# kaistmm/Audio-Mamba-AuM

Hardware: AMD Instinct MI355X
Metric: clips/sec/node AuM-Base 128x1024 fwd+bwd (higher is better)
Workload: dtype bf16; 1 GPU; AuM-Base (d_model=768, 24 Fo-Bi blocks, d_state=16, 92.1M params) 128-mel x 1024-frame clips, L=513 tokens, fwd+bwd+Adam, bf16 autocast / fp32 master weights, input = 160000-sample waveforms through the one-launch HIP frontend (log-mel + 16x16 patch embedding + position rows); per_gpu_batch=64, global_batch=64, parallelism=dp1

## Files before the change

audio-mamba-aum_amd/aum_hip/__init__.py:

```python
import ctypes as C
import math
import os

import torch

_HERE = os.path.dirname(os.path.abspath(__file__))
_SO = os.path.join(_HERE, "libaum_hip.so")

AUM_F32, AUM_BF16, AUM_F16 = 0, 1, 2
SCAN_SOFTPLUS, SCAN_REVERSE, SCAN_GENERIC, SCAN_ROWPAIR, SCAN_ACCUMULATE = 1, 2, 4, 8, 16
CONV_SILU, CONV_REVERSE = 1, 2
_DT = {torch.float32: AUM_F32, torch.bfloat16: AUM_BF16, torch.float16: AUM_F16}
_ERR = {-1: "AUM_E_NULL", -2: "AUM_E_SHAPE", -3: "AUM_E_DTYPE", -4: "AUM_E_UNSUPPORTED", -5: "AUM_E_WORKSPACE",
        -6: "AUM_E_LAUNCH"}

_i64, _i32, _u32, _vp, _fp = C.c_int64, C.c_int32, C.c_uint32, C.c_void_p, C.c_void_p
ABI_VERSION = 13


class _Debug:

    def __init__(self):
        self.ablate = 0
        self.rowpair = False
        self.no_ckpt = False
        self.no_accumulate = False
        self.no_lane_ckpt = False
        self.proj_splits = 0
        self.torch_sums = False
        self.sums_one_by_one = False
        if os.environ.get("AUM_DEBUG") == "1":
            self.ablate = int(os.environ.get("AUM_ABLATE", "0"))
            self.rowpair = os.environ.get("AUM_SCAN_ROWPAIR") == "1"
            self.no_ckpt = os.environ.get("AUM_SCAN_NO_CKPT") == "1"
            self.no_accumulate = os.environ.get("AUM_SCAN_NO_ACCUMULATE") == "1"
            self.no_lane_ckpt = os.environ.get("AUM_SCAN_NO_LANE_CKPT") == "1"
            self.torch_sums = os.environ.get("AUM_TORCH_SUMS") == "1"
            self.sums_one_by_one = os.environ.get("AUM_SUMS_ONE_BY_ONE") == "1"


debug = _Debug()


class ScanFwdArgs(C.Structure):
    _fields_ = ([(n, _vp) for n in ("u", "delta", "z", "B", "C", "A", "A_b", "D", "delta_bias", "out", "out_pre",
                                    "last_state", "workspace")]
                + [(n, _i64) for n in ("workspace_bytes", "u_bs", "u_ds", "delta_bs", "delta_ds", "z_bs", "z_ds", "B_bs",
                                       "B_ns", "C_bs", "C_ns", "out_bs", "out_ds")]
                + [(n, _i32) for n in ("batch", "dim", "len", "dstate", "dtype")] + [("flags", _u32), ("x_ck", _vp), ("x_lane", _vp)])


class ScanBwdArgs(C.Structure):
    _fields_ = ([(n, _vp) for n in ("u", "delta", "z", "B", "C", "dout", "out_pre", "A", "A_b", "D", "delta_bias", "du",
                                    "ddelta", "dz", "dA", "dA_b", "dB", "dC", "dD", "ddelta_bias", "workspace")]
                + [(n, _i64) for n in ("workspace_bytes", "u_bs", "u_ds", "delta_bs", "delta_ds", "z_bs", "z_ds", "B_bs",
                                       "B_ns", "C_bs", "C_ns", "dout_bs", "dout_ds", "out_bs", "out_ds", "du_bs", "du_ds",
                                       "ddelta_bs", "ddelta_ds", "dz_bs", "dz_ds", "dB_bs", "dB_ns", "dC_bs", "dC_ns")]
                + [(n, _i32) for n in ("batch", "dim", "len", "dstate", "dtype")] + [("flags", _u32), ("x_ck", _vp), ("x_lane", _vp)])


class ScanTmFwdArgs(C.Structure):
    _fields_ = ([(n, _vp) for n in ("u", "delta", "z", "B", "C", "A", "A_b", "D", "delta_bias", "out", "out_pre", "ckpt")]
                + [(n, _i64) for n in ("u_bs", "u_ts", "delta_bs", "delta_ts", "z_bs", "z_ts", "B_bs", "B_ts", "C_bs", "C_ts",
# ... 64 lines not shown
    _fields_ = ([("fbank", FbankArgs)] + [(n, _vp) for n in ("weight", "bias", "pos", "cls_row", "tokens", "patches")]
                + [("tokens_bs", _i64)] + [(n, _i32) for n in ("dim", "cls_pos", "dtype", "out_dtype")] + [("flags", _u32)])


class ProjArgs(C.Structure):
    _fields_ = ([(n, _vp) for n in ("act", "w_x", "w_dt", "x_dbl", "out_act", "dB", "dC")]
                + [(n, _i64) for n in ("dB_bs", "dB_ns", "dC_bs", "dC_ns", "ntok")]
                + [(n, _i32) for n in ("dim", "dt_rank", "dstate", "len", "dtype", "w_ld")])


class ProjWArgs(C.Structure):
    _fields_ = ([(n, _vp) for n in ("x", "y", "out")] + [("ntok", _i64)]
                + [(n, _i32) for n in ("dim", "nrows", "nsplit", "transpose_out", "dtype")])


class GemmArgs(C.Structure):
    _fields_ = ([(n, _vp) for n in ("a", "b", "c")] + [(n, _i32) for n in ("m", "n", "k", "lda", "ldb", "ldc", "dtype")] + [("flags", _u32)])


class XdtBwdArgs(C.Structure):
    _fields_ = ([(n, _vp) for n in ("ddelta", "dbc", "wdt_t", "wx_t", "du", "dx_dbl")] + [("ntok", _i64)]
                + [(n, _i32) for n in ("dim", "rank", "ncols", "ldd", "lddbc", "ldwdt", "ldwx", "ldu", "ldx", "dtype")])


class GemmWArgs(C.Structure):
    _fields_ = [("y", C.c_void_p), ("x", C.c_void_p), ("part", C.c_void_p), ("t", C.c_int64), ("ldy", C.c_int64), ("ldx", C.c_int64),
                ("n", C.c_int32), ("k", C.c_int32), ("splits", C.c_int32), ("dtype", C.c_int32)]


SUM_MAX_JOBS = 8


class SumJob(C.Structure):
    _fields_ = [("src", C.c_void_p), ("dst", C.c_void_p), ("outer", C.c_int64), ("inner", C.c_int64), ("tr_cols", C.c_int32), ("reserved", C.c_int32)]


class ConvUpdateArgs(C.Structure):
    _fields_ = [("x", C.c_void_p), ("conv_state", C.c_void_p), ("weight", C.c_void_p), ("bias", C.c_void_p), ("out", C.c_void_p),
                ("batch", C.c_int32), ("dim", C.c_int32), ("width", C.c_int32), ("dtype", C.c_int32), ("flags", C.c_uint32)]


class StateUpdateArgs(C.Structure):
    _fields_ = [("state", C.c_void_p), ("x", C.c_void_p), ("dt", C.c_void_p), ("z", C.c_void_p), ("B", C.c_void_p), ("C", C.c_void_p),
                ("A", C.c_void_p), ("D", C.c_void_p), ("dt_bias", C.c_void_p), ("out", C.c_void_p),
                ("batch", C.c_int32), ("dim", C.c_int32), ("dstate", C.c_int32), ("dtype", C.c_int32), ("flags", C.c_uint32)]


class DtProjArgs(C.Structure):
    _fields_ = ([(n, _vp) for n in ("x", "w", "out")] + [("ntok", _i64)] + [(n, _i32) for n in ("dim", "rank", "ldx", "ldw", "ldo", "dtype")])


class XdtArgs(C.Structure):
    _fields_ = ([(n, _vp) for n in ("u", "wx", "wdt", "x_dbl", "delta")] + [("ntok", _i64)]
                + [(n, _i32) for n in ("dim", "rank", "ncols", "ldu", "ldwx", "ldwdt", "ldx", "ldd", "dtype")])


EXPORTS = ["aum_gemm_tn", "aum_dtproj_tm_fwd", "aum_xdt_tm_fwd", "aum_proj_fwd", "aum_proj_bwd_data", "aum_proj_bwd_weight", "aum_proj_bwd_weight_splits", "aum_fbank_fwd", "aum_frontend_tokens_fwd", "aum_abi_version", "aum_selective_scan_fwd", "aum_selective_scan_bwd", "aum_scan_max_single_pass_len",
           "aum_selective_scan_workspace_bytes", "aum_selective_scan_ckpt_bytes", "aum_selective_scan_lane_ckpt_bytes", "aum_causal_conv1d_fwd", "aum_causal_conv1d_bwd", "aum_rmsnorm_fwd",
           "aum_rmsnorm_bwd", "aum_rmsnorm_bwd_partials", "aum_selftest_wave_scan", "aum_hbm_copy", "aum_sum_rows", "aum_sum_rows_multi",
           "aum_scan_tm_fwd", "aum_scan_tm_nck", "aum_scan_tm_ckpt_rows", "aum_scan_tm_bwd", "aum_scan_tm_workspace_bytes", "aum_scan_tm_seg_fwd", "aum_scan_tm_seg_bwd",
           "aum_scan_tm_seg_carry_bytes", "aum_scan_tm_seg_workspace_bytes", "aum_selftest_wave_sum32",
           "aum_conv1d_tm_fwd", "aum_conv1d_tm_bwd", "aum_conv1d_tm_nparts", "aum_gemm_wgrad", "aum_xdt_tm_bwd", "aum_causal_conv1d_update", "aum_selective_state_update", "aum_cast_bank", "aum_rmsnorm_bwd_partial_rows",
           "aum_stft_logmel_fwd", "aum_spec_time_warp"]


class Lib:

    def __init__(self, path, host=False):
        if not os.path.exists(path):
            raise ImportError(
                f"{path} not found: the HIP extension is not built.  Run `python audio-mamba-aum_amd/csrc/build.py` "
                "(hipcc, gfx950).  There is no CPU fallback on the product path.")
        self.path, self.host = path, host
        self.c = C.CDLL(path)
        for name in EXPORTS:
            getattr(self.c, name)
        self.c.aum_selective_scan_workspace_bytes.restype = _i64
        self.c.aum_selective_scan_workspace_bytes.argtypes = [_i32] * 6
        for n in ("aum_selective_scan_fwd", "aum_selective_scan_bwd", "aum_causal_conv1d_fwd", "aum_causal_conv1d_bwd",
                  "aum_rmsnorm_fwd", "aum_rmsnorm_bwd"):
            getattr(self.c, n).argtypes = [_vp, _vp]
        self.c.aum_scan_tm_fwd.argtypes = [_vp, _vp]
        self.c.aum_scan_tm_bwd.argtypes = [_vp, _vp]
        self.c.aum_scan_tm_seg_fwd.argtypes = [_vp, _vp]
        self.c.aum_scan_tm_seg_bwd.argtypes = [_vp, _vp]
        self.c.aum_scan_tm_nck.argtypes = [_i32]
        self.c.aum_scan_tm_ckpt_rows.argtypes = [_i32]
        self.c.aum_conv1d_tm_fwd.argtypes = [_vp, _vp]
        self.c.aum_conv1d_tm_bwd.argtypes = [_vp, _vp]
        self.c.aum_conv1d_tm_nparts.argtypes = [_i32, _i32]
        self.c.aum_gemm_tn.argtypes = [_vp, _vp]
        self.c.aum_gemm_wgrad.argtypes = [_vp, _vp]
        self.c.aum_causal_conv1d_update.argtypes = [_vp, _vp]
        self.c.aum_selective_state_update.argtypes = [_vp, _vp]
        self.c.aum_dtproj_tm_fwd.argtypes = [_vp, _vp]
        self.c.aum_xdt_tm_fwd.argtypes = [_vp, _vp]
        self.c.aum_xdt_tm_bwd.argtypes = [_vp, _vp]
        self.c.aum_scan_tm_workspace_bytes.restype = _i64
        self.c.aum_scan_tm_workspace_bytes.argtypes = [_i32] * 5
        for fn in (self.c.aum_scan_tm_seg_carry_bytes, self.c.aum_scan_tm_seg_workspace_bytes):
            fn.restype = _i64
            fn.argtypes = [_i32] * 6
        self.c.aum_fbank_fwd.argtypes = [_vp, _vp]
        self.c.aum_frontend_tokens_fwd.argtypes = [_vp, _vp]
        self.c.aum_stft_logmel_fwd.argtypes = [_vp, _vp]
        self.c.aum_spec_time_warp.argtypes = [_vp, _vp]
        for n in ("aum_proj_fwd", "aum_proj_bwd_data", "aum_proj_bwd_weight"):
# ... 252 lines not shown
        a.dz_bs, a.dz_ds = dz.stride(0), dz.stride(1)
    a.B_bs, a.B_ns, a.C_bs, a.C_ns = B.stride(0), B.stride(1), C.stride(0), C.stride(1)
    a.dout_bs, a.dout_ds = dout.stride(0), dout.stride(1)
    a.du_bs, a.du_ds = du.stride(0), du.stride(1)
    a.ddelta_bs, a.ddelta_ds = ddelta.stride(0), ddelta.stride(1)
    a.dB_bs, a.dB_ns, a.dC_bs, a.dC_ns = dB.stride(0), dB.stride(1), dC.stride(0), dC.stride(1)
    a.batch, a.dim, a.len, a.dstate, a.dtype = batch, dim, length, dstate, _DT[u.dtype]
    a.flags = ((SCAN_SOFTPLUS if delta_softplus else 0) | (SCAN_REVERSE if reverse else 0) | (SCAN_GENERIC if generic else 0)
               | (SCAN_ROWPAIR if rowpair or debug.rowpair else 0)
               | (SCAN_ACCUMULATE if acc else 0)
               | (debug.ablate << 16))
    _launch(lib.c.aum_selective_scan_bwd, a, u, lib, "scan_bwd_bidir" if A_b is not None else "scan_bwd",
            (batch, dim, length, dstate, u.element_size(), True))
    return dict(du=du, ddelta=ddelta, dA=dA, dA_b=dA_b, dB=dB, dC=dC, dD=dD, dz=dz, ddelta_bias=dbias)


SCAN_TM_CK = 8


def scan_tm_supported(dim, dstate):
    return dstate == 16 and dim % 64 == 0


def _tm3(t, name, last):
    if t.dim() != 3 or t.shape[2] != last or (t.stride(2) != 1 and last != 1):
        raise RuntimeError(f"{name}: expected (batch, len, {last}) with the last axis contiguous (token-major)")
    ts = t.stride(1) if t.shape[1] > 1 else last
    bs = t.stride(0) if t.shape[0] > 1 else ts * t.shape[1]
    return bs, ts


def scan_tm_ckpt(batch, length, dim, dstate, bidir, device, lib=None, dtype=torch.float32):
    lib = lib or get()
    nck = int(lib.c.aum_scan_tm_nck(length))
    rows = int(lib.c.aum_scan_tm_ckpt_rows(_DT[dtype])) if dstate == 16 else dstate
    return torch.empty((2 if bidir else 1, batch, max(nck, 1), rows, dim), dtype=torch.float32, device=device)


SCAN_TM_MAX_SEGMENTS = 32


def scan_tm_segments(batch, dim, length, bidir, training=False, nsimd=None, device=None):
    nsimd = 4 * cu_count(device) if nsimd is None else nsimd
    per_dir = batch * (dim // 64)
    waves = per_dir * (2 if bidir else 1)
    if per_dir <= 0 or waves * 2 > nsimd or length < 1024:
        return 1
    want = -(-nsimd * 3 // per_dir)
    seg = min(want, length // 128, SCAN_TM_MAX_SEGMENTS)
    return seg if seg >= 2 else 1


def scan_tm_fwd(u, delta, A, B, C, D=None, z=None, delta_bias=None, delta_softplus=False, reverse=False, A_b=None,
                want_out_pre=False, ckpt=None, out=None, lib=None, segments=1):
    lib = lib or get()
    batch, length, dim = u.shape
    dstate = A.shape[1]
    for t in (u, delta, z, B, C):
        lib.check_tensor(t)
    if u.dtype not in _DT or delta.dtype != u.dtype or (z is not None and z.dtype != u.dtype):
        raise RuntimeError("u, delta, z must share one dtype in {fp32, bf16, fp16}")
    if B.dtype != u.dtype or C.dtype != u.dtype:
        raise RuntimeError("B, C must have u's dtype")
    A, A_b, D, delta_bias = _f32c(A), _f32c(A_b), _f32c(D), _f32c(delta_bias)
    a = ScanTmFwdArgs()
    a.u_bs, a.u_ts = _tm3(u, "u", dim)
    a.delta_bs, a.delta_ts = _tm3(delta, "delta", dim)
    if z is not None:
        a.z_bs, a.z_ts = _tm3(z, "z", dim)
    a.B_bs, a.B_ts = _tm3(B, "B", dstate)
    a.C_bs, a.C_ts = _tm3(C, "C", dstate)
    if out is None:
        out = torch.empty((batch, length, dim), dtype=u.dtype, device=u.device)
    out_pre = torch.empty((batch, length, dim), dtype=u.dtype, device=u.device) if want_out_pre else None
    a.out_bs, a.out_ts = _tm3(out, "out", dim)
    if out_pre is not None:
        a.pre_bs, a.pre_ts = _tm3(out_pre, "out_pre", dim)
    a.u, a.delta, a.z, a.B, a.C = _ptr(u), _ptr(delta), _ptr(z), _ptr(B), _ptr(C)
    a.A, a.A_b, a.D, a.delta_bias = _ptr(A), _ptr(A_b), _ptr(D), _ptr(delta_bias)
    a.out, a.out_pre = _ptr(out), _ptr(out_pre)
    if ckpt is not None:
        assert ckpt.dtype == torch.float32 and ckpt.is_contiguous()
        rows = int(lib.c.aum_scan_tm_ckpt_rows(_DT[u.dtype])) if dstate == 16 else dstate
        assert ckpt.numel() >= (2 if A_b is not None else 1) * batch * max(int(lib.c.aum_scan_tm_nck(length)), 1) * rows * dim, "ckpt too small"
        lib.check_tensor(ckpt)
        a.ckpt = _ptr(ckpt)
    a.batch, a.dim, a.len, a.dstate, a.dtype = batch, dim, length, dstate, _DT[u.dtype]
    a.flags = (SCAN_SOFTPLUS if delta_softplus else 0) | (SCAN_REVERSE if reverse else 0)
    if segments > 1:
        sa = ScanTmSegFwdArgs()
        sa.base = a
        sa.segments = int(segments)
        sa.carry_bytes = int(lib.c.aum_scan_tm_seg_carry_bytes(batch, dim, length, dstate, int(A_b is not None), int(segments)))
        if sa.carry_bytes <= 0:
            raise RuntimeError(f"scan_tm_fwd: segments={segments} not supported for this shape")
        carry = torch.empty((sa.carry_bytes // 4,), dtype=torch.float32, device=u.device)
        sa.carry = _ptr(carry)
        _launch(lib.c.aum_scan_tm_seg_fwd, sa, u, lib, "scan_tm_seg_fwd_bidir" if A_b is not None else "scan_tm_seg_fwd",
                (batch, dim, length, dstate, u.element_size(), want_out_pre, int(segments)))
        return out, out_pre
    _launch(lib.c.aum_scan_tm_fwd, a, u, lib, "scan_tm_fwd_bidir" if A_b is not None else "scan_tm_fwd",
            (batch, dim, length, dstate, u.element_size(), want_out_pre))
    return out, out_pre


def scan_tm_bwd(u, delta, A, B, C, D, z, delta_bias, dout, out_pre, ckpt, delta_softplus=False, reverse=False, A_b=None, dz_out=None,
                lib=None, segments=1, want_dA_xA=False, param_out=None):
    lib = lib or get()
    batch, length, dim = u.shape
    dstate = A.shape[1]
    dev = u.device
    for t in (u, delta, z, B, C, dout, out_pre, ckpt):
        lib.check_tensor(t)
    if u.dtype not in _DT:
        raise RuntimeError("u must be fp32, bf16 or fp16")
    for name, t in (("delta", delta), ("z", z), ("B", B), ("C", C), ("dout", dout), ("out_pre", out_pre), ("dz_out", dz_out)):
        if t is not None and t.dtype != u.dtype:
            raise RuntimeError(f"{name} must have u's dtype ({u.dtype}), got {t.dtype}")
    for name, t in (("delta", delta), ("z", z), ("dout", dout), ("out_pre", out_pre), ("dz_out", dz_out)):
        if t is not None and tuple(t.shape) != (batch, length, dim):
            raise RuntimeError(f"{name}: expected shape {(batch, length, dim)}, got {tuple(t.shape)}")
    if z is not None and out_pre is None:
        raise RuntimeError("out_pre (the forward's pre-gate sum) is required when z is given")
    A, A_b, D, delta_bias = _f32c(A), _f32c(A_b), _f32c(D), _f32c(delta_bias)
    bidir = A_b is not None
    if ckpt is None or ckpt.dtype != torch.float32 or not ckpt.is_contiguous():
        raise RuntimeError("ckpt: the contiguous fp32 tensor scan_tm_fwd filled")
    rows_ = int(lib.c.aum_scan_tm_ckpt_rows(_DT[u.dtype])) if dstate == 16 else dstate
    if ckpt.numel() < (2 if bidir else 1) * batch * max(int(lib.c.aum_scan_tm_nck(length)), 1) * rows_ * dim:
        raise RuntimeError("ckpt too small for this launch")
    du = torch.empty((batch, length, dim), dtype=u.dtype, device=dev)
    ddelta = torch.empty((batch, length, dim), dtype=u.dtype, device=dev)
    dz = None
    if z is not None:
        dz = dz_out if dz_out is not None else torch.empty((batch, length, dim), dtype=u.dtype, device=dev)
    f32 = dict(dtype=torch.float32, device=dev)
    dBC = torch.empty((batch, length, 2 * dstate), **f32)
    po = param_out or {}
    dA = torch.empty((dim, dstate), **f32)
    dA_b = torch.empty((dim, dstate), **f32) if bidir else None
    dD = _sum_out(po.get("dD"), (dim,), dev) if D is not None else None
    dbias = _sum_out(po.get("ddelta_bias"), (dim,), dev) if delta_bias is not None else None
    dA_xA = _sum_out(po.get("dA_xA"), (dim, dstate), dev) if want_dA_xA else None
    dA_b_xA = _sum_out(po.get("dA_b_xA"), (dim, dstate), dev) if want_dA_xA and bidir else None
    if segments > 1:
        ws_bytes = int(lib.c.aum_scan_tm_seg_workspace_bytes(batch, dim, length, dstate, int(bidir), int(segments)))
        if ws_bytes <= 0:
            raise RuntimeError(f"scan_tm_bwd: segments={segments} not supported for this shape")
    else:
        ws_bytes = int(lib.c.aum_scan_tm_workspace_bytes(batch, dim, length, dstate, int(bidir)))
    ws = torch.empty((max(ws_bytes, 4) // 4,), **f32)
    a = ScanTmBwdArgs()
    a.u, a.delta, a.z, a.B, a.C, a.dout, a.out_pre = map(_ptr, (u, delta, z, B, C, dout, out_pre))
    a.A, a.A_b, a.D, a.delta_bias, a.ckpt = _ptr(A), _ptr(A_b), _ptr(D), _ptr(delta_bias), _ptr(ckpt)
    a.du, a.ddelta, a.dz = _ptr(du), _ptr(ddelta), _ptr(dz)
    a.dA, a.dA_b, a.dBC, a.dD, a.ddelta_bias = map(_ptr, (dA, dA_b, dBC, dD, dbias))
    a.dA_xA, a.dA_b_xA = _ptr(dA_xA), _ptr(dA_b_xA)
    a.workspace, a.workspace_bytes = _ptr(ws), ws_bytes
    a.u_bs, a.u_ts = _tm3(u, "u", dim)
    a.delta_bs, a.delta_ts = _tm3(delta, "delta", dim)
    a.B_bs, a.B_ts = _tm3(B, "B", dstate)
    a.C_bs, a.C_ts = _tm3(C, "C", dstate)
    a.dout_bs, a.dout_ts = _tm3(dout, "dout", dim)
    a.du_bs, a.du_ts = _tm3(du, "du", dim)
    a.ddelta_bs, a.ddelta_ts = _tm3(ddelta, "ddelta", dim)
    if z is not None:
        a.z_bs, a.z_ts = _tm3(z, "z", dim)
        a.pre_bs, a.pre_ts = _tm3(out_pre, "out_pre", dim)
        a.dz_bs, a.dz_ts = _tm3(dz, "dz", dim)
    a.batch, a.dim, a.len, a.dstate, a.dtype = batch, dim, length, dstate, _DT[u.dtype]
    a.flags = (SCAN_SOFTPLUS if delta_softplus else 0) | (SCAN_REVERSE if reverse else 0)
    if segments > 1:
        sa = ScanTmSegBwdArgs()
        sa.base = a
        sa.segments = int(segments)
        _launch(lib.c.aum_scan_tm_seg_bwd, sa, u, lib, "scan_tm_seg_bwd_bidir" if bidir else "scan_tm_seg_bwd",
                (batch, dim, length, dstate, u.element_size(), True, int(segments)))
    else:
        _launch(lib.c.aum_scan_tm_bwd, a, u, lib, "scan_tm_bwd_bidir" if bidir else "scan_tm_bwd", (batch, dim, length, dstate, u.element_size(), True))
    return dict(du=du, ddelta=ddelta, dz=dz, dBC=dBC, dA=dA, dA_b=dA_b, dD=dD, ddelta_bias=dbias, dA_xA=dA_xA, dA_b_xA=dA_b_xA, _ws=ws)


GEMM_BN, GEMM_BK = 256, 64


_dev_cu = {}


def cu_count(device=None):
    if not torch.cuda.is_available():
        return 256
    idx = torch.cuda.current_device() if device is None else torch.device(device).index
    idx = torch.cuda.current_device() if idx is None else idx
    n = _dev_cu.get(idx)
    if n is None:
        n = _dev_cu[idx] = int(torch.cuda.get_device_properties(idx).multi_processor_count)
    return n


def gemm_wgrad_splits(n, k, ncu=None, device=None):
    ncu = cu_count(device) if ncu is None else ncu
    tiles = (n // 256) * max(1, k // 256)
    return max(1, min(64, ncu // max(tiles, 1)))


def gemm_wgrad_supported(y, x, splits=None):
    if not (y.dim() == 2 and x.dim() == 2 and y.dtype == x.dtype and y.dtype in (torch.bfloat16, torch.float16) and y.shape[0] == x.shape[0]
            and y.stride(1) == 1 and x.stride(1) == 1 and y.shape[1] % 256 == 0 and (x.shape[1] % 256 == 0 or x.shape[1] in (48, 80))
            and y.stride(0) % 8 == 0 and y.stride(0) >= y.shape[1] and x.stride(0) >= x.shape[1]
            and x.stride(0) % 8 == 0 and y.data_ptr() % 16 == 0 and x.data_ptr() % 16 == 0 and y.shape[0] > 0):
        return False
    splits = splits or gemm_wgrad_splits(y.shape[1], x.shape[1], device=y.device if y.is_cuda else None)
    if not 0 < splits <= 64:
        return False
    chunk = (-(-y.shape[0] // splits) + 63) // 64 * 64
    return chunk * y.stride(0) * 2 < (1 << 31) and chunk * x.stride(0) * 2 < (1 << 31)


def gemm_wgrad(y, x, splits=None, lib=None, partials=False, out=None):
    lib = lib or get()
    t, n = y.shape
    k = x.shape[1]
    splits = splits or gemm_wgrad_splits(n, k, device=y.device if y.is_cuda else None)
    if not gemm_wgrad_supported(y, x, splits):
# ... 97 lines not shown
    lib.check_tensor(w)
    if not dtproj_tm_supported(x_dbl, rank, w):
        raise RuntimeError(f"dtproj_tm_fwd: unsupported operands {tuple(x_dbl.shape)} {x_dbl.dtype}, rank {rank}, weight {tuple(w.shape)} {w.dtype}")
    ntok, dim = x_dbl.shape[0], w.shape[0]
    out = torch.empty((ntok, dim), dtype=x_dbl.dtype, device=x_dbl.device)
    a = DtProjArgs()
    a.x, a.w, a.out = _ptr(x_dbl), _ptr(w), _ptr(out)
    a.ntok, a.dim, a.rank, a.ldx, a.ldw, a.ldo, a.dtype = ntok, dim, rank, x_dbl.stride(0), w.stride(0), dim, _DT[x_dbl.dtype]
    _launch(lib.c.aum_dtproj_tm_fwd, a, x_dbl, lib, "dtproj_tm_fwd", (ntok, dim, rank))
    return out


XDT_COLS, XDT_MAX_DIM = 80, 1536
XDT_COLS_FWD = (80, 56)


def xdt_tm_supported(u, wx, wdt):
    if not (u.dim() == 2 and wx.dim() == 2 and wdt.dim() == 2 and u.dtype == wx.dtype == wdt.dtype and u.dtype in (torch.bfloat16, torch.float16)):
        return False
    dim, rank = u.shape[1], wdt.shape[1]
    ok_t = lambda t: t.stride(1) == 1 and t.stride(0) % 8 == 0 and t.data_ptr() % 16 == 0
    return (wx.shape[0] in XDT_COLS_FWD and wx.shape[1] == dim and wdt.shape[0] == dim and dim % 256 == 0 and dim <= XDT_MAX_DIM and rank % 8 == 0
            and rank <= 64 and rank <= wx.shape[0]
            and ok_t(u) and ok_t(wx) and ok_t(wdt))


def xdt_tm_bwd_supported(ddelta, dbc, wdt_t, wx_t, du):
    if not (ddelta.dim() == 2 and du.shape == ddelta.shape and ddelta.dtype == du.dtype == wdt_t.dtype == wx_t.dtype
            and ddelta.dtype in (torch.bfloat16, torch.float16) and dbc.dtype == torch.float32 and dbc.dim() == 2):
        return False
    ntok, dim = ddelta.shape
    ok_t = lambda t, m=8: t.stride(1) == 1 and t.stride(0) % m == 0 and t.data_ptr() % 16 == 0
    return (wx_t.shape == (dim, XDT_COLS) and wdt_t.shape == (XDT_COLS - 32, dim) and dbc.shape == (ntok, 32) and dim % 256 == 0
            and dim <= XDT_MAX_DIM and ok_t(ddelta) and ok_t(du) and ok_t(wdt_t) and ok_t(wx_t) and ok_t(dbc, 4))


def xdt_tm_bwd(ddelta, dbc, wdt_t, wx_t, du, lib=None):
    lib = lib or get()
    for t in (ddelta, dbc, wdt_t, wx_t, du):
        lib.check_tensor(t)
    if not xdt_tm_bwd_supported(ddelta, dbc, wdt_t, wx_t, du):
        raise RuntimeError(f"xdt_tm_bwd: unsupported operands {tuple(ddelta.shape)} {ddelta.dtype}, {tuple(dbc.shape)}, {tuple(wdt_t.shape)}, {tuple(wx_t.shape)}")
    ntok, dim = ddelta.shape
    dx_dbl = torch.empty((ntok, XDT_COLS), dtype=ddelta.dtype, device=ddelta.device)
    a = XdtBwdArgs()
    a.ddelta, a.dbc, a.wdt_t, a.wx_t, a.du, a.dx_dbl = _ptr(ddelta), _ptr(dbc), _ptr(wdt_t), _ptr(wx_t), _ptr(du), _ptr(dx_dbl)
    a.ntok, a.dim, a.rank, a.ncols = ntok, dim, XDT_COLS - 32, XDT_COLS
    a.ldd, a.lddbc, a.ldwdt, a.ldwx, a.ldu, a.ldx = ddelta.stride(0), dbc.stride(0), wdt_t.stride(0), wx_t.stride(0), du.stride(0), XDT_COLS
    a.dtype = _DT[ddelta.dtype]
    _launch(lib.c.aum_xdt_tm_bwd, a, ddelta, lib, "xdt_tm_bwd", (ntok, dim))
    return dx_dbl


def xdt_tm_fwd(u, wx, wdt, lib=None):
    lib = lib or get()
    for t in (u, wx, wdt):
        lib.check_tensor(t)
    if not xdt_tm_supported(u, wx, wdt):
        raise RuntimeError(f"xdt_tm_fwd: unsupported operands {tuple(u.shape)} {u.dtype}, {tuple(wx.shape)}, {tuple(wdt.shape)}")
    ntok, dim = u.shape
    rank = wdt.shape[1]
    ncols = wx.shape[0]
    x_dbl = torch.empty((ntok, ncols), dtype=u.dtype, device=u.device)
    delta = torch.empty((ntok, dim), dtype=u.dtype, device=u.device)
    a = XdtArgs()
    a.u, a.wx, a.wdt, a.x_dbl, a.delta = _ptr(u), _ptr(wx), _ptr(wdt), _ptr(x_dbl), _ptr(delta)
    a.ntok, a.dim, a.rank, a.ncols = ntok, dim, rank, ncols
    a.ldu, a.ldwx, a.ldwdt, a.ldx, a.ldd, a.dtype = u.stride(0), wx.stride(0), wdt.stride(0), ncols, dim, _DT[u.dtype]
    _launch(lib.c.aum_xdt_tm_fwd, a, u, lib, "xdt_tm_fwd", (ntok, dim, rank))
    return x_dbl, delta


def conv1d_tm_supported(x, width):
    if x.dim() != 3 or x.dtype not in _DT or width > 4 or (x.stride(2) != 1 and x.shape[2] != 1):
        return False
    es = x.element_size()
    bs, ts = _tm3(x, "x", x.shape[2])
    return x.shape[2] % (16 // es) == 0 and x.data_ptr() % 16 == 0 and (ts * es) % 16 == 0 and (bs * es) % 16 == 0


def _al16(t):
    return t if t is None or t.data_ptr() % 16 == 0 else t.clone()


def conv1d_tm_fwd(x, weight, bias=None, silu=True, reverse=False, lib=None):
    lib = lib or get()
    lib.check_tensor(x)
    batch, length, dim = x.shape
    weight = _al16(_f32c(weight.reshape(dim, -1)))
    bias = _al16(_f32c(bias))
    y = torch.empty((batch, length, dim), dtype=x.dtype, device=x.device)
    a = ConvTmArgs()
    a.x, a.weight, a.bias, a.y = _ptr(x), _ptr(weight), _ptr(bias), _ptr(y)
    a.x_bs, a.x_ts = _tm3(x, "x", dim)
    a.y_bs, a.y_ts = _tm3(y, "y", dim)
    a.batch, a.dim, a.len, a.width, a.dtype = batch, dim, length, weight.shape[1], _DT[x.dtype]
    a.flags = (CONV_SILU if silu else 0) | (CONV_REVERSE if reverse else 0)
    _launch(lib.c.aum_conv1d_tm_fwd, a, x, lib, "conv_tm_fwd", (batch, dim, length, x.element_size()))
    return y


def conv1d_tm_bwd(x, weight, bias, dy, silu=True, reverse=False, dx_out=None, lib=None, partials=False):
    lib = lib or get()
    lib.check_tensor(x)
    batch, length, dim = x.shape
    weight = _al16(_f32c(weight.reshape(dim, -1)))
    bias = _al16(_f32c(bias))
    width = weight.shape[1]
    dy = dy if dy.stride(2) == 1 else dy.contiguous()
    dx = dx_out if dx_out is not None else torch.empty((batch, length, dim), dtype=x.dtype, device=x.device)
    nparts = int(lib.c.aum_conv1d_tm_nparts(batch, length))
    f32 = dict(dtype=torch.float32, device=x.device)
    dw_part = torch.empty((nparts, dim, width), **f32)
    db_part = torch.empty((nparts, dim), **f32) if bias is not None else None
    a = ConvTmArgs()
    a.x, a.dy, a.weight, a.bias, a.dx, a.dw_part, a.db_part = map(_ptr, (x, dy, weight, bias, dx, dw_part, db_part))
    a.x_bs, a.x_ts = _tm3(x, "x", dim)
    a.dy_bs, a.dy_ts = _tm3(dy, "dy", dim)
    a.dx_bs, a.dx_ts = _tm3(dx, "dx", dim)
    a.batch, a.dim, a.len, a.width, a.dtype = batch, dim, length, width, _DT[x.dtype]
    a.flags = (CONV_SILU if silu else 0) | (CONV_REVERSE if reverse else 0)
# ... 401 lines not shown
```

audio-mamba-aum_amd/csrc/aum_api_tm.inc:

```
#include "scan_tm_kernels.h"
#include "conv_tm_kernels.h"

namespace aum {

#ifndef AUM_SCANT_FWD_MINW
#define AUM_SCANT_FWD_MINW 3
#endif

int scan_tm_fwd_f32(const AumScanTmFwdArgs& a, aum_stream_t s);
int scan_tm_fwd_bf16(const AumScanTmFwdArgs& a, aum_stream_t s);
int scan_tm_fwd_f16(const AumScanTmFwdArgs& a, aum_stream_t s);
int scan_tm_bwd_f32(const AumScanTmBwdArgs& a, const ScanTBwdOut& wo, aum_stream_t s);
int scan_tm_bwd_bf16(const AumScanTmBwdArgs& a, const ScanTBwdOut& wo, aum_stream_t s);
int scan_tm_bwd_f16(const AumScanTmBwdArgs& a, const ScanTBwdOut& wo, aum_stream_t s);
int scan_tm_seg_fwd_f32(const AumScanTmFwdArgs& a, const ScanTSeg& sg, int phase, aum_stream_t s);
int scan_tm_seg_fwd_bf16(const AumScanTmFwdArgs& a, const ScanTSeg& sg, int phase, aum_stream_t s);
int scan_tm_seg_fwd_f16(const AumScanTmFwdArgs& a, const ScanTSeg& sg, int phase, aum_stream_t s);
int scan_tm_seg_bwd_f32(const AumScanTmBwdArgs& a, const ScanTBwdOut& wo, const ScanTSeg& sg, int phase, aum_stream_t s);
int scan_tm_seg_bwd_bf16(const AumScanTmBwdArgs& a, const ScanTBwdOut& wo, const ScanTSeg& sg, int phase, aum_stream_t s);
int scan_tm_seg_bwd_f16(const AumScanTmBwdArgs& a, const ScanTBwdOut& wo, const ScanTSeg& sg, int phase, aum_stream_t s);

struct ScanTWs { int64_t dbc, dA, dD, dbias, carry, total, trace; int nparts, ndir; };
static ScanTWs scant_ws_layout(int batch, int dim, int len, int dstate, bool bidir, int nseg = 1) {
    ScanTWs w;
// ... 63 lines not shown
template <class T, int PHASE, bool SP, bool HAS_Z, bool HAS_PRE>
__global__ __launch_bounds__(SCANT_NW * 64, AUM_SCANT_FWD_MINW) void k_scant_seg_fwd(AumScanTmFwdArgs a, ScanTSeg sg) {
    __shared__ __attribute__((aligned(16))) float lds[SCANT_NW * scant_lds_wave_floats<T>()];
    scant_seg_fwd<T, PHASE, SP, HAS_Z, HAS_PRE>(a, sg, (int)blockIdx.x, lds);
}
#endif
template <class T, int PHASE, bool SP, bool HAS_Z, bool HAS_PRE> static int launch_scant_seg_fwd(const AumScanTmFwdArgs& a, const ScanTSeg& sg, aum_stream_t s) {
    const int grid = (a.batch * (a.dim / WAVE) * sg.nseg * sg.ndl + SCANT_NW - 1) / SCANT_NW;
#ifdef AUM_EMU
    (void)s;
    std::vector<float> lds(SCANT_NW * scant_lds_wave_floats<T>());
    for (int wg = 0; wg < grid; ++wg) scant_seg_fwd<T, PHASE, SP, HAS_Z, HAS_PRE>(a, sg, wg, lds.data());
#else
    hipLaunchKernelGGL((k_scant_seg_fwd<T, PHASE, SP, HAS_Z, HAS_PRE>), dim3((unsigned)grid), dim3(SCANT_NW * 64), 0, s, a, sg);
#endif
    return launch_status();
}
template <class T> static int scan_tm_seg_fwd_t(const AumScanTmFwdArgs& a, const ScanTSeg& sg, int phase, aum_stream_t s) {
    const bool sp = (a.flags & AUM_SCAN_SOFTPLUS) != 0;
    if (phase == 3) return sp ? launch_scant_seg_fwd<T, 3, true, false, false>(a, sg, s) : launch_scant_seg_fwd<T, 3, false, false, false>(a, sg, s);
    if (phase == 4) {
        if (a.z) return sp ? launch_scant_seg_fwd<T, 4, true, true, false>(a, sg, s) : launch_scant_seg_fwd<T, 4, false, true, false>(a, sg, s);
        return sp ? launch_scant_seg_fwd<T, 4, true, false, false>(a, sg, s) : launch_scant_seg_fwd<T, 4, false, false, false>(a, sg, s);
    }
    const int key = (sp ? 4 : 0) | (a.z ? 2 : 0) | (a.out_pre ? 1 : 0);
    switch (phase * 8 + key) {
#define AUM_TMS(P, K) case (P) * 8 + (K): return launch_scant_seg_fwd<T, P, ((K) & 4) != 0, ((K) & 2) != 0, ((K) & 1) != 0>(a, sg, s);
#define AUM_TMS8(P) AUM_TMS(P, 0) AUM_TMS(P, 1) AUM_TMS(P, 2) AUM_TMS(P, 3) AUM_TMS(P, 4) AUM_TMS(P, 5) AUM_TMS(P, 6) AUM_TMS(P, 7)
        AUM_TMS8(0) AUM_TMS8(1) AUM_TMS8(2)
#undef AUM_TMS8
#undef AUM_TMS
    }
    return AUM_E_UNSUPPORTED;
}
#if AUM_HAS_DTYPE(0)
int scan_tm_fwd_f32(const AumScanTmFwdArgs& a, aum_stream_t s) { return scan_tm_fwd_t<float>(a, s); }
int scan_tm_seg_fwd_f32(const AumScanTmFwdArgs& a, const ScanTSeg& sg, int phase, aum_stream_t s) { return scan_tm_seg_fwd_t<float>(a, sg, phase, s); }
#endif
#if AUM_HAS_DTYPE(1)
int scan_tm_fwd_bf16(const AumScanTmFwdArgs& a, aum_stream_t s) { return scan_tm_fwd_t<bf16_t>(a, s); }
int scan_tm_seg_fwd_bf16(const AumScanTmFwdArgs& a, const ScanTSeg& sg, int phase, aum_stream_t s) { return scan_tm_seg_fwd_t<bf16_t>(a, sg, phase, s); }
#endif
#if AUM_HAS_DTYPE(2)
int scan_tm_fwd_f16(const AumScanTmFwdArgs& a, aum_stream_t s) { return scan_tm_fwd_t<f16_t>(a, s); }
int scan_tm_seg_fwd_f16(const AumScanTmFwdArgs& a, const ScanTSeg& sg, int phase, aum_stream_t s) { return scan_tm_seg_fwd_t<f16_t>(a, sg, phase, s); }
#endif
#endif

#ifndef AUM_SCANT_BWD_MINW
#define AUM_SCANT_BWD_MINW 2
#endif
#if AUM_API_PART == 6 || AUM_API_PART == 0
#ifndef AUM_EMU
template <class T, bool SP, bool HAS_Z, bool BIDIR>
__global__ __launch_bounds__(SCANT_NW * 64, AUM_SCANT_BWD_MINW) void k_scant_bwd(AumScanTmBwdArgs a, ScanTBwdOut wo) {
    __shared__ __attribute__((aligned(16))) float lds[SCANT_NW * scant_bwd_lds_wave_floats<T>()];
#ifdef AUM_SCANT_TRACE
    unsigned long long* tr = wo.trace + ((size_t)blockIdx.x * SCANT_NW + threadIdx.x / 64) * 16;
    const unsigned long long t_begin = __builtin_amdgcn_s_memrealtime();
    unsigned long long tacc[12] = {0, 0, 0, 0, 0, 0, 0, 0, 0, 0, 0, 0};
    scant_bwd<T, SP, HAS_Z, BIDIR>(a, wo, (int)blockIdx.x, lds, tacc);
    if ((threadIdx.x & 63) == 0) {
        tr[0] = __builtin_amdgcn_s_getreg((31 << 11) | 4);
        tr[1] = __builtin_amdgcn_s_getreg((31 << 11) | 20);
        tr[2] = t_begin;
        tr[3] = __builtin_amdgcn_s_memrealtime();
        for (int k = 0; k < 12; ++k) tr[4 + k] = tacc[k];
    }
#else
    scant_bwd<T, SP, HAS_Z, BIDIR>(a, wo, (int)blockIdx.x, lds);
#endif
}
#endif
template <class T, bool SP, bool HAS_Z, bool BIDIR> static int launch_scant_bwd(const AumScanTmBwdArgs& a, const ScanTBwdOut& wo, aum_stream_t s) {
    const int grid = scant_bwd_wgs<BIDIR>(a.batch * (a.dim / WAVE));
#ifdef AUM_EMU
    (void)s;
    std::vector<float> lds(SCANT_NW * scant_bwd_lds_wave_floats<T>());
    for (int wg = 0; wg < grid; ++wg) scant_bwd<T, SP, HAS_Z, BIDIR>(a, wo, wg, lds.data());
#else
    hipLaunchKernelGGL((k_scant_bwd<T, SP, HAS_Z, BIDIR>), dim3((unsigned)grid), dim3(SCANT_NW * 64), 0, s, a, wo);
#endif
    return launch_status();
}
template <class T> static int scan_tm_bwd_t(const AumScanTmBwdArgs& a, const ScanTBwdOut& wo, aum_stream_t s) {
    const int key = ((a.flags & AUM_SCAN_SOFTPLUS) ? 4 : 0) | (a.z ? 2 : 0) | (a.A_b ? 1 : 0);
    switch (key) {
#define AUM_TMB(K) case K: return launch_scant_bwd<T, ((K) & 4) != 0, ((K) & 2) != 0, ((K) & 1) != 0>(a, wo, s);
        AUM_TMB(0) AUM_TMB(1) AUM_TMB(2) AUM_TMB(3) AUM_TMB(4) AUM_TMB(5) AUM_TMB(6) AUM_TMB(7)
#undef AUM_TMB
    }
    return AUM_E_UNSUPPORTED;
}
#ifndef AUM_EMU
template <class T, int PHASE, bool SP, bool HAS_Z>
__global__ __launch_bounds__(SCANT_NW * 64, AUM_SCANT_BWD_MINW) void k_scant_seg_bwd(AumScanTmBwdArgs a, ScanTBwdOut wo, ScanTSeg sg) {
    __shared__ __attribute__((aligned(16))) float lds[SCANT_NW * scant_bwd_lds_wave_floats<T>()];
    scant_seg_bwd<T, PHASE, SP, HAS_Z>(a, wo, sg, (int)blockIdx.x, lds);
}
#endif
template <class T, int PHASE, bool SP, bool HAS_Z>
static int launch_scant_seg_bwd(const AumScanTmBwdArgs& a, const ScanTBwdOut& wo, const ScanTSeg& sg, aum_stream_t s) {
    const int grid = (a.batch * (a.dim / WAVE) * sg.nseg + SCANT_NW - 1) / SCANT_NW;
#ifdef AUM_EMU
    (void)s;
    std::vector<float> lds(SCANT_NW * scant_bwd_lds_wave_floats<T>());
    for (int wg = 0; wg < grid; ++wg) scant_seg_bwd<T, PHASE, SP, HAS_Z>(a, wo, sg, wg, lds.data());
#else
    hipLaunchKernelGGL((k_scant_seg_bwd<T, PHASE, SP, HAS_Z>), dim3((unsigned)grid), dim3(SCANT_NW * 64), 0, s, a, wo, sg);
#endif
    return launch_status();
}
template <class T> static int scan_tm_seg_bwd_t(const AumScanTmBwdArgs& a, const ScanTBwdOut& wo, const ScanTSeg& sg, int phase, aum_stream_t s) {
    const int key = ((a.flags & AUM_SCAN_SOFTPLUS) ? 2 : 0) | (a.z ? 1 : 0);
    switch (phase * 4 + key) {
#define AUM_TMS(P, K) case (P) * 4 + (K): return launch_scant_seg_bwd<T, P, ((K) & 2) != 0, ((K) & 1) != 0>(a, wo, sg, s);
#define AUM_TMS4(P) AUM_TMS(P, 0) AUM_TMS(P, 1) AUM_TMS(P, 2) AUM_TMS(P, 3)
        AUM_TMS4(0) AUM_TMS4(1) AUM_TMS4(2)
#undef AUM_TMS4
#undef AUM_TMS
    }
    return AUM_E_UNSUPPORTED;
}
#if AUM_HAS_DTYPE(0)
int scan_tm_bwd_f32(const AumScanTmBwdArgs& a, const ScanTBwdOut& wo, aum_stream_t s) { return scan_tm_bwd_t<float>(a, wo, s); }
int scan_tm_seg_bwd_f32(const AumScanTmBwdArgs& a, const ScanTBwdOut& wo, const ScanTSeg& sg, int phase, aum_stream_t s) { return scan_tm_seg_bwd_t<float>(a, wo, sg, phase, s); }
#endif
#if AUM_HAS_DTYPE(1)
int scan_tm_bwd_bf16(const AumScanTmBwdArgs& a, const ScanTBwdOut& wo, aum_stream_t s) { return scan_tm_bwd_t<bf16_t>(a, wo, s); }
int scan_tm_seg_bwd_bf16(const AumScanTmBwdArgs& a, const ScanTBwdOut& wo, const ScanTSeg& sg, int phase, aum_stream_t s) { return scan_tm_seg_bwd_t<bf16_t>(a, wo, sg, phase, s); }
#endif
#if AUM_HAS_DTYPE(2)
int scan_tm_bwd_f16(const AumScanTmBwdArgs& a, const ScanTBwdOut& wo, aum_stream_t s) { return scan_tm_bwd_t<f16_t>(a, wo, s); }
int scan_tm_seg_bwd_f16(const AumScanTmBwdArgs& a, const ScanTBwdOut& wo, const ScanTSeg& sg, int phase, aum_stream_t s) { return scan_tm_seg_bwd_t<f16_t>(a, wo, sg, phase, s); }
#endif
#endif

}

#if AUM_API_PART == 3 || AUM_API_PART == 0
AUM_API int32_t aum_scan_tm_nck(int32_t len) { return len > 0 ? scant_nck(len) : 0; }
AUM_API int32_t aum_scan_tm_ckpt_rows(int32_t dtype) {
    return dtype == AUM_F32 ? scant_ck_rows<float>() : (dtype == AUM_BF16 || dtype == AUM_F16) ? scant_ck_rows<bf16_t>() : 0;
}

static int scan_tm_fwd_check(const AumScanTmFwdArgs* a) {
    if (!a) return AUM_E_NULL;
    if (!a->u || !a->delta || !a->B || !a->C || !a->A || !a->out) return AUM_E_NULL;
    if (a->batch <= 0 || a->dim <= 0 || a->len <= 0 || a->dstate <= 0) return AUM_E_SHAPE;
    if (a->dtype < 0 || a->dtype > 2) return AUM_E_DTYPE;
    if (!scant_supported(a->dim, a->dstate)) return AUM_E_UNSUPPORTED;
    if (a->A_b && (a->flags & AUM_SCAN_REVERSE)) return AUM_E_UNSUPPORTED;
    if (a->dtype != AUM_F32) {
        if ((a->B_bs | a->B_ts | a->C_bs | a->C_ts) & 1) return AUM_E_UNSUPPORTED;
        if ((((uintptr_t)a->B) | ((uintptr_t)a->C)) & 3) return AUM_E_UNSUPPORTED;
    }
    {
        const int64_t es = a->dtype == AUM_F32 ? 4 : 2, lim = ((int64_t)1 << 31) - 1;
        const int64_t ts[] = {a->u_ts, a->delta_ts, a->z ? a->z_ts : 0, a->out_ts, a->out_pre ? a->pre_ts : 0, a->B_ts, a->C_ts};
        for (int64_t t : ts)
            if (t < 0 || t * es * a->len > lim) return AUM_E_UNSUPPORTED;
        if ((int64_t)scant_nck(a->len) * a->dstate * a->dim * 4 > lim) return AUM_E_UNSUPPORTED;
        const uintptr_t ptrs = (uintptr_t)a->u | (uintptr_t)a->delta | (uintptr_t)a->z | (uintptr_t)a->out | (uintptr_t)a->out_pre;
        const int64_t strides = a->u_bs | a->u_ts | a->delta_bs | a->delta_ts | (a->z ? (a->z_bs | a->z_ts) : 0) | a->out_bs | a->out_ts |
                                (a->out_pre ? (a->pre_bs | a->pre_ts) : 0);
        if ((ptrs & 15) || ((strides * es) & 15)) return AUM_E_UNSUPPORTED;
    }
    return AUM_OK;
}
AUM_API int aum_scan_tm_fwd(const AumScanTmFwdArgs* a, void* stream) {
    const int rc = scan_tm_fwd_check(a);
    if (rc != AUM_OK) return rc;
    aum_stream_t s = (aum_stream_t)stream;
    switch (a->dtype) {
        case AUM_F32: return scan_tm_fwd_f32(*a, s);
        case AUM_BF16: return scan_tm_fwd_bf16(*a, s);
        default: return scan_tm_fwd_f16(*a, s);
    }
}
static int scan_tm_seg_fwd_any(const AumScanTmFwdArgs& a, const ScanTSeg& sg, int phase, aum_stream_t s) {
    switch (a.dtype) {
        case AUM_F32: return scan_tm_seg_fwd_f32(a, sg, phase, s);
        case AUM_BF16: return scan_tm_seg_fwd_bf16(a, sg, phase, s);
        default: return scan_tm_seg_fwd_f16(a, sg, phase, s);
    }
}
AUM_API int64_t aum_scan_tm_seg_carry_bytes(int32_t batch, int32_t dim, int32_t len, int32_t dstate, int32_t bidirectional, int32_t segments) {
    if (batch <= 0 || dim <= 0 || len <= 0 || segments < 2 || !scant_supported(dim, dstate)) return 0;
    return scant_seg_carry_floats(batch, dim, segments, bidirectional != 0) * (int64_t)sizeof(float);
}
AUM_API int aum_scan_tm_seg_fwd(const AumScanTmSegFwdArgs* sa, void* stream) {
    if (!sa) return AUM_E_NULL;
    const AumScanTmFwdArgs* a = &sa->base;
    const int rc = scan_tm_fwd_check(a);
    if (rc != AUM_OK) return rc;
    if (sa->segments < 2 || sa->segments > AUM_SCAN_TM_MAX_SEGMENTS) return AUM_E_SHAPE;
    if (!sa->carry) return AUM_E_NULL;
    const bool bidir = a->A_b != nullptr;
    if (sa->carry_bytes < scant_seg_carry_floats(a->batch, a->dim, sa->segments, bidir) * (int64_t)sizeof(float)) return AUM_E_WORKSPACE;
    aum_stream_t s = (aum_stream_t)stream;
    ScanTSeg sg;
    sg.carry = sa->carry;
    sg.nseg = sa->segments;
    sg.seg_len = scant_seg_len(a->len, sa->segments);
    sg.dir0 = 0;
    sg.ndl = bidir ? 2 : 1;
    int r = scan_tm_seg_fwd_any(*a, sg, 3, s);
    if (r != AUM_OK) return r;
    sg.ndl = 1;
    if (!bidir) return scan_tm_seg_fwd_any(*a, sg, 0, s);
    r = scan_tm_seg_fwd_any(*a, sg, 1, s);
    if (r != AUM_OK) return r;
    sg.dir0 = 1;
    return scan_tm_seg_fwd_any(*a, sg, 2, s);
}
AUM_API int64_t aum_scan_tm_workspace_bytes(int32_t batch, int32_t dim, int32_t len, int32_t dstate, int32_t bidirectional) {
    if (batch <= 0 || dim <= 0 || len <= 0 || dstate <= 0 || !scant_supported(dim, dstate)) return 0;
    return scant_ws_layout(batch, dim, len, dstate, bidirectional != 0).total * (int64_t)sizeof(float);
}

struct ScanTReduceArgs {
    const float* ws;
    float *dBC, *dA, *dA_b, *dD, *dbias;
    const float *A, *A_b;
    float *dAx, *dAx_b;
    int64_t o_dA, o_dD, o_dbias;
    int32_t batch, pbatch, dim, len, dstate, nparts, ndir;
    int32_t nsum;
};
#ifndef AUM_EMU
__global__ __launch_bounds__(256) void k_scant_bwd_reduce(ScanTReduceArgs a) {
    const int64_t ntok = (int64_t)a.batch * a.len;
    const int k4 = 2 * a.dstate / 4;
    const int64_t n_bc = ntok * k4;
    const int64_t n_a = (int64_t)a.ndir * a.dim * a.dstate;
    const int64_t n_d = 2 * (int64_t)a.dim;
    for (int64_t i = (int64_t)blockIdx.x * blockDim.x + threadIdx.x; i < n_bc + n_a + n_d; i += (int64_t)gridDim.x * blockDim.x) {
        if (i < n_bc) {
            const int64_t tok = i / k4;
            const int c = (int)(i % k4);
            const float4* src = reinterpret_cast<const float4*>(a.ws) + (tok * a.nparts) * k4 + c;
            float4 acc = make_float4(0.f, 0.f, 0.f, 0.f);
#pragma unroll 8
            for (int q = 0; q < a.nsum; ++q) {
                const float4 v = src[(int64_t)q * k4];
                acc.x += v.x; acc.y += v.y; acc.z += v.z; acc.w += v.w;
            }
            reinterpret_cast<float4*>(a.dBC)[i] = acc;
        } else if (i < n_bc + n_a) {
            const int64_t r = i - n_bc;
            const int d = (int)(r / ((int64_t)a.dim * a.dstate));
            const int64_t en = r % ((int64_t)a.dim * a.dstate);
            const int e = (int)(en / a.dstate), n = (int)(en % a.dstate);
            const float* src = a.ws + a.o_dA + (int64_t)d * a.pbatch * a.dstate * a.dim + (int64_t)n * a.dim + e;
            float acc = 0.f;
#pragma unroll 16
            for (int b = 0; b < a.pbatch; ++b) acc += src[(int64_t)b * a.dstate * a.dim];
            (d ? a.dA_b : a.dA)[en] = acc;
            float* px = d ? a.dAx_b : a.dAx;
            if (px) px[en] = acc * (d ? a.A_b : a.A)[en];
        } else {
            const int64_t r = i - n_bc - n_a;
            const bool is_bias = r >= a.dim;
            const int e = (int)(r % a.dim);
            float* dst = is_bias ? a.dbias : a.dD;
            if (!dst) continue;
            const float* src = a.ws + (is_bias ? a.o_dbias : a.o_dD) + e;
            float acc = 0.f;
#pragma unroll 16
            for (int q = 0; q < a.ndir * a.pbatch; ++q) acc += src[(int64_t)q * a.dim];
            dst[e] = acc;
        }
    }
}
#endif
static int scant_reduce_launch(const ScanTReduceArgs& a, aum_stream_t s) {
#ifdef AUM_EMU
    (void)s;
    const int64_t ntok = (int64_t)a.batch * a.len;
    const int K = 2 * a.dstate;
    for (int64_t tok = 0; tok < ntok; ++tok)
        for (int k = 0; k < K; ++k) {
            float acc = 0.f;
            for (int q = 0; q < a.nsum; ++q) acc += a.ws[(tok * a.nparts + q) * K + k];
            a.dBC[tok * K + k] = acc;
        }
    for (int d = 0; d < a.ndir; ++d)
        for (int e = 0; e < a.dim; ++e)
            for (int n = 0; n < a.dstate; ++n) {
                float acc = 0.f;
                for (int b = 0; b < a.pbatch; ++b) acc += a.ws[a.o_dA + (((int64_t)d * a.pbatch + b) * a.dstate + n) * a.dim + e];
                (d ? a.dA_b : a.dA)[(int64_t)e * a.dstate + n] = acc;
                float* px = d ? a.dAx_b : a.dAx;
                if (px) px[(int64_t)e * a.dstate + n] = acc * (d ? a.A_b : a.A)[(int64_t)e * a.dstate + n];
            }
    for (int e = 0; e < a.dim; ++e) {
        float accD = 0.f, accb = 0.f;
        for (int q = 0; q < a.ndir * a.pbatch; ++q) {
            accD += a.ws[a.o_dD + (int64_t)q * a.dim + e];
            accb += a.ws[a.o_dbias + (int64_t)q * a.dim + e];
        }
        if (a.dD) a.dD[e] = accD;
        if (a.dbias) a.dbias[e] = accb;
    }
#else
    hipLaunchKernelGGL(k_scant_bwd_reduce, dim3(2048), dim3(256), 0, s, a);
#endif
    return launch_status();
}

static int scan_tm_bwd_any(const AumScanTmBwdArgs* a, int nseg, void* stream) {
    if (!a) return AUM_E_NULL;
    if (!a->u || !a->delta || !a->B || !a->C || !a->A || !a->dout || !a->ckpt) return AUM_E_NULL;
    if (!a->du || !a->ddelta || !a->dA || !a->dBC || !a->workspace) return AUM_E_NULL;
    if (a->z && (!a->out_pre || !a->dz)) return AUM_E_NULL;
    if (a->A_b && !a->dA_b) return AUM_E_NULL;
    if (a->batch <= 0 || a->dim <= 0 || a->len <= 0 || a->dstate <= 0) return AUM_E_SHAPE;
    if (a->dtype < 0 || a->dtype > 2) return AUM_E_DTYPE;
    if (!scant_supported(a->dim, a->dstate)) return AUM_E_UNSUPPORTED;
    if (a->A_b && (a->flags & AUM_SCAN_REVERSE)) return AUM_E_UNSUPPORTED;
    const int64_t es = a->dtype == AUM_F32 ? 4 : 2, lim = ((int64_t)1 << 31) - 1;
    if (a->dtype != AUM_F32) {
        if ((a->B_bs | a->B_ts | a->C_bs | a->C_ts) & 1) return AUM_E_UNSUPPORTED;
        if ((((uintptr_t)a->B) | ((uintptr_t)a->C)) & 3) return AUM_E_UNSUPPORTED;
    }
    {
        const int64_t ts[] = {a->u_ts, a->delta_ts, a->z ? a->z_ts : 0, a->dout_ts, a->z ? a->pre_ts : 0, a->du_ts, a->ddelta_ts, a->z ? a->dz_ts : 0,
                              a->B_ts, a->C_ts};
        for (int64_t t : ts)
            if (t < 0 || t * es * a->len > lim) return AUM_E_UNSUPPORTED;
        const uintptr_t ptrs = (uintptr_t)a->u | (uintptr_t)a->delta | (uintptr_t)a->z | (uintptr_t)a->dout | (uintptr_t)a->out_pre | (uintptr_t)a->du |
                               (uintptr_t)a->ddelta | (uintptr_t)a->dz;
        const int64_t strides = a->u_bs | a->u_ts | a->delta_bs | a->delta_ts | a->dout_bs | a->dout_ts | a->du_bs | a->du_ts | a->ddelta_bs | a->ddelta_ts |
                                (a->z ? (a->z_bs | a->z_ts | a->pre_bs | a->pre_ts | a->dz_bs | a->dz_ts) : 0);
        if ((ptrs & 15) || ((strides * es) & 15)) return AUM_E_UNSUPPORTED;
    }
    const bool bidir = a->A_b != nullptr;
    if (nseg != 1 && (nseg < 2 || nseg > AUM_SCAN_TM_MAX_SEGMENTS)) return AUM_E_SHAPE;
    const ScanTWs L = scant_ws_layout(a->batch, a->dim, a->len, a->dstate, bidir, nseg);
    if (a->workspace_bytes < L.total * (int64_t)sizeof(float)) return AUM_E_WORKSPACE;
    if ((int64_t)a->len * L.nparts * 2 * a->dstate * 4 > lim || (int64_t)scant_nck(a->len) * a->dstate * a->dim * 4 > lim) return AUM_E_UNSUPPORTED;
    float* ws = (float*)a->workspace;
    ScanTBwdOut wo;
    wo.dbc = ws + L.dbc;
    wo.dA = ws + L.dA;
    wo.dD = ws + L.dD;
    wo.dbias = ws + L.dbias;
    wo.nparts = L.nparts;
    wo.carry = ws + L.carry;
    wo.trace = nullptr;
#ifdef AUM_SCANT_TRACE
    wo.trace = reinterpret_cast<unsigned long long*>(ws + L.trace);
#endif
    aum_stream_t s = (aum_stream_t)stream;
    int rc = AUM_OK;
    if (nseg == 1) {
        switch (a->dtype) {
            case AUM_F32: rc = scan_tm_bwd_f32(*a, wo, s); break;
            case AUM_BF16: rc = scan_tm_bwd_bf16(*a, wo, s); break;
            default: rc = scan_tm_bwd_f16(*a, wo, s); break;
        }
    } else {
        ScanTSeg sg;
        sg.carry = ws + L.carry;
        sg.nseg = nseg;
        sg.seg_len = scant_seg_len(a->len, nseg);
        sg.dir0 = 0;
        sg.ndl = bidir ? 2 : 1;
        {
            AumScanTmFwdArgs f = {};
            f.u = a->dout; f.u_bs = a->dout_bs; f.u_ts = a->dout_ts;
            f.delta = a->delta; f.delta_bs = a->delta_bs; f.delta_ts = a->delta_ts;
            f.z = a->z; f.z_bs = a->z_bs; f.z_ts = a->z_ts;
            f.B = a->C; f.B_bs = a->C_bs; f.B_ts = a->C_ts;
            f.C = a->C; f.C_bs = a->C_bs; f.C_ts = a->C_ts;
            f.A = a->A; f.A_b = a->A_b; f.delta_bias = a->delta_bias;
            f.out = a->du; f.out_bs = a->du_bs; f.out_ts = a->du_ts;
            f.batch = a->batch; f.dim = a->dim; f.len = a->len; f.dstate = a->dstate; f.dtype = a->dtype; f.flags = a->flags;
            rc = scan_tm_seg_fwd_any(f, sg, 4, s);
            if (rc != AUM_OK) return rc;
        }
        sg.ndl = 1;
        for (int d = 0; d < (bidir ? 2 : 1) && rc == AUM_OK; ++d) {
            sg.dir0 = d;
            const int phase = bidir ? 1 + d : 0;
            switch (a->dtype) {
                case AUM_F32: rc = scan_tm_seg_bwd_f32(*a, wo, sg, phase, s); break;
                case AUM_BF16: rc = scan_tm_seg_bwd_bf16(*a, wo, sg, phase, s); break;
                default: rc = scan_tm_seg_bwd_f16(*a, wo, sg, phase, s); break;
            }
        }
    }
    if (rc != AUM_OK) return rc;
    ScanTReduceArgs r;
    r.ws = ws;
    r.dBC = a->dBC; r.dA = a->dA; r.dA_b = a->dA_b; r.dD = a->D ? a->dD : nullptr; r.dbias = a->delta_bias ? a->ddelta_bias : nullptr;
    r.o_dA = L.dA; r.o_dD = L.dD; r.o_dbias = L.dbias;
    r.A = a->A; r.A_b = a->A_b; r.dAx = a->dA_xA; r.dAx_b = a->A_b ? a->dA_b_xA : nullptr;
    r.batch = a->batch; r.pbatch = a->batch * nseg; r.dim = a->dim; r.len = a->len; r.dstate = a->dstate; r.nparts = L.nparts; r.ndir = L.ndir; r.nsum = scant_dbc_rows_to_sum(L.nparts, bidir);
    return scant_reduce_launch(r, s);
}
AUM_API int aum_scan_tm_bwd(const AumScanTmBwdArgs* a, void* stream) { return scan_tm_bwd_any(a, 1, stream); }
AUM_API int aum_scan_tm_seg_bwd(const AumScanTmSegBwdArgs* sa, void* stream) {
    if (!sa) return AUM_E_NULL;
    if (sa->segments < 2) return AUM_E_SHAPE;
    return scan_tm_bwd_any(&sa->base, sa->segments, stream);
}
AUM_API int64_t aum_scan_tm_seg_workspace_bytes(int32_t batch, int32_t dim, int32_t len, int32_t dstate, int32_t bidirectional, int32_t segments) {
    if (batch <= 0 || dim <= 0 || len <= 0 || dstate <= 0 || segments < 2 || segments > AUM_SCAN_TM_MAX_SEGMENTS || !scant_supported(dim, dstate)) return 0;
    return scant_ws_layout(batch, dim, len, dstate, bidirectional != 0, segments).total * (int64_t)sizeof(float);
}
#ifndef AUM_EMU
template <class T, bool SILU> AUM_GLOBAL void k_convt_fwd(AumConvTmArgs a) { convt_fwd_wave<T, SILU>(a, (int)blockIdx.x); }
template <class T, bool SILU> AUM_GLOBAL void k_convt_bwd(AumConvTmArgs a) { convt_bwd_wave<T, SILU>(a, (int)blockIdx.x); }
#endif
template <class T, bool SILU> static int convt_launch(const AumConvTmArgs& a, bool bwd, aum_stream_t s) {
    const int grid = bwd ? a.batch * convt_chunks<true>(a.len) * convt_cblocks<T, true>(a.dim) : a.batch * convt_chunks<false>(a.len) * convt_cblocks<T, false>(a.dim);
#ifdef AUM_EMU
    (void)s;
    for (int wg = 0; wg < grid; ++wg) {
        if (bwd) convt_bwd_wave<T, SILU>(a, wg); else convt_fwd_wave<T, SILU>(a, wg);
    }
#else
    if (bwd) AUM_LAUNCH((k_convt_bwd<T, SILU>), grid, 0, s, a); else AUM_LAUNCH((k_convt_fwd<T, SILU>), grid, 0, s, a);
#endif
    return launch_status();
}
template <class T> static int convt_dispatch_t(const AumConvTmArgs& a, bool bwd, aum_stream_t s) {
    return (a.flags & AUM_CONV_SILU) ? convt_launch<T, true>(a, bwd, s) : convt_launch<T, false>(a, bwd, s);
}
static int convt_dispatch(const AumConvTmArgs* a, bool bwd, void* stream) {
    if (!a || !a->x || !a->weight) return AUM_E_NULL;
    if (bwd ? (!a->dy || !a->dx || !a->dw_part) : !a->y) return AUM_E_NULL;
    if (bwd && a->bias && !a->db_part) return AUM_E_NULL;
    if (a->batch <= 0 || a->dim <= 0 || a->len <= 0 || a->width <= 0) return AUM_E_SHAPE;
    if (a->dtype < 0 || a->dtype > 2) return AUM_E_DTYPE;
    if (a->width > CONVT_W) return AUM_E_UNSUPPORTED;
    const int64_t es = a->dtype == AUM_F32 ? 4 : 2;
    if (a->dim % (16 / es)) return AUM_E_UNSUPPORTED;
    const uintptr_t ptrs = (uintptr_t)a->x | (uintptr_t)(bwd ? a->dy : a->y) | (uintptr_t)(bwd ? a->dx : a->y) | (uintptr_t)a->weight |
                           (uintptr_t)a->bias;
    const int64_t strides = a->x_bs | a->x_ts | (bwd ? (a->dy_bs | a->dy_ts | a->dx_bs | a->dx_ts) : (a->y_bs | a->y_ts));
    if ((ptrs & 15) || ((strides * es) & 15)) return AUM_E_UNSUPPORTED;
    const int64_t lim = (int64_t)1 << 31;
    const int64_t ts = a->x_ts > (bwd ? (a->dy_ts > a->dx_ts ? a->dy_ts : a->dx_ts) : a->y_ts) ? a->x_ts : (bwd ? (a->dy_ts > a->dx_ts ? a->dy_ts : a->dx_ts) : a->y_ts);
    if ((int64_t)a->len * ts * es >= lim) return AUM_E_UNSUPPORTED;
    aum_stream_t s = (aum_stream_t)stream;
    switch (a->dtype) {
        case AUM_F32: return convt_dispatch_t<float>(*a, bwd, s);
// ... 9 lines not shown
```

audio-mamba-aum_amd/csrc/gemm.hip:

```cpp
#include <atomic>
#include "gemm_kernels.h"
#include "gemm_ps_kernels.h"
#include "dtproj_kernels.h"
#include "xdt_kernels.h"
#include "decode_kernels.h"
#include "cast_kernels.h"

static int cu_count() {
    static std::atomic<int> ncu_of[64];
    int dev = 0;
    if (hipGetDevice(&dev) != hipSuccess || dev < 0 || dev >= 64) return 0;
    int ncu = ncu_of[dev].load(std::memory_order_relaxed);
    if (!ncu) {
        if (hipDeviceGetAttribute(&ncu, hipDeviceAttributeMultiprocessorCount, dev) != hipSuccess || ncu <= 0) return 0;
        ncu_of[dev].store(ncu, std::memory_order_relaxed);
    }
    return ncu;
}

extern "C" int aum_gemm_tn(const AumGemmArgs* p, void* stream) {
    const int rc = aumg::gemm_check(p);
    if (rc != AUM_OK) return rc;
    const AumGemmArgs& g = *p;
    const int tiles = (g.m + aumg::BM - 1) / aumg::BM * (g.n / aumg::BN);
// ... 11 lines not shown
        const int grid = L.nitems < ncu ? L.nitems : ncu;
        if (g.dtype == AUM_BF16) hipLaunchKernelGGL(aumg::k_gemm_tn_ps<true>, dim3(grid), dim3(aumg::THREADS), 0, s, L);
        else hipLaunchKernelGGL(aumg::k_gemm_tn_ps<false>, dim3(grid), dim3(aumg::THREADS), 0, s, L);
        return hipGetLastError() == hipSuccess ? AUM_OK : AUM_E_LAUNCH;
    }
    const bool bf = g.dtype == AUM_BF16;
    if (flags & AUM_GEMM_PIPELINED) {
        if (bf) hipLaunchKernelGGL((aumg::k_gemm_tn<true, 2>), dim3(tiles), dim3(aumg::THREADS), 0, s, g);
        else hipLaunchKernelGGL((aumg::k_gemm_tn<false, 2>), dim3(tiles), dim3(aumg::THREADS), 0, s, g);
    } else {
        if (bf) hipLaunchKernelGGL((aumg::k_gemm_tn<true, 0>), dim3(tiles), dim3(aumg::THREADS), 0, s, g);
        else hipLaunchKernelGGL((aumg::k_gemm_tn<false, 0>), dim3(tiles), dim3(aumg::THREADS), 0, s, g);
    }
    return hipGetLastError() == hipSuccess ? AUM_OK : AUM_E_LAUNCH;
}

extern "C" int aum_gemm_wgrad(const AumGemmWArgs* p, void* stream) {
    const int rc = aumg::gemm_wgrad_check(p);
    if (rc != AUM_OK) return rc;
    const AumGemmWArgs& g = *p;
    const bool skinny = g.k % 256 != 0;
    const int nitems = (g.n / 256) * (skinny ? 1 : g.k / 256) * g.splits;
    const int grid = (nitems + 7) / 8 * 8;
    hipStream_t s = static_cast<hipStream_t>(stream);
    (void)hipGetLastError();
    const bool bf = g.dtype == AUM_BF16;
    if (skinny && g.k == 48) {
        if (bf) hipLaunchKernelGGL((aumg::k_gemm_wgrad_skinny<true, 3>), dim3(grid), dim3(aumg::THREADS), 0, s, g);
        else hipLaunchKernelGGL((aumg::k_gemm_wgrad_skinny<false, 3>), dim3(grid), dim3(aumg::THREADS), 0, s, g);
    } else if (skinny) {
        if (bf) hipLaunchKernelGGL((aumg::k_gemm_wgrad_skinny<true, 5>), dim3(grid), dim3(aumg::THREADS), 0, s, g);
        else hipLaunchKernelGGL((aumg::k_gemm_wgrad_skinny<false, 5>), dim3(grid), dim3(aumg::THREADS), 0, s, g);
    } else if (bf) hipLaunchKernelGGL(aumg::k_gemm_wgrad<true>, dim3(grid), dim3(aumg::THREADS), 0, s, g);
    else hipLaunchKernelGGL(aumg::k_gemm_wgrad<false>, dim3(grid), dim3(aumg::THREADS), 0, s, g);
    return hipGetLastError() == hipSuccess ? AUM_OK : AUM_E_LAUNCH;
}

extern "C" int aum_dtproj_tm_fwd(const AumDtProjArgs* p, void* stream) {
    const int rc = aumd::dtproj_check(p);
    if (rc != AUM_OK) return rc;
    const AumDtProjArgs& g = *p;
    const int64_t nwaves = (g.ntok + aumd::TOK_PER_WAVE - 1) / aumd::TOK_PER_WAVE;
    const dim3 grid((unsigned)((nwaves + aumd::WAVES - 1) / aumd::WAVES)), block(aumd::WAVES * 64);
    hipStream_t s = static_cast<hipStream_t>(stream);
    const bool bf = g.dtype == AUM_BF16, one = g.rank <= 32;
    if (bf && one) hipLaunchKernelGGL((aumd::k_dtproj_tm<true, 1>), grid, block, 0, s, g);
    else if (bf) hipLaunchKernelGGL((aumd::k_dtproj_tm<true, 2>), grid, block, 0, s, g);
    else if (one) hipLaunchKernelGGL((aumd::k_dtproj_tm<false, 1>), grid, block, 0, s, g);
    else hipLaunchKernelGGL((aumd::k_dtproj_tm<false, 2>), grid, block, 0, s, g);
    return hipGetLastError() == hipSuccess ? AUM_OK : AUM_E_LAUNCH;
}


template <int NW, int NC> static void xdt_launch_nc(const AumXdtArgs& g, hipStream_t s) {
    const dim3 grid((unsigned)((g.ntok + NW * XDT_TOK_W - 1) / (NW * XDT_TOK_W))), block(NW * 64);
    const bool bf = g.dtype == AUM_BF16, one = g.rank <= 32;
    if (bf && one) hipLaunchKernelGGL((aumx::k_xdt_tm_fwd<true, 1, NW, NC>), grid, block, 0, s, g);
    else if (bf) hipLaunchKernelGGL((aumx::k_xdt_tm_fwd<true, 2, NW, NC>), grid, block, 0, s, g);
    else if (one) hipLaunchKernelGGL((aumx::k_xdt_tm_fwd<false, 1, NW, NC>), grid, block, 0, s, g);
    else hipLaunchKernelGGL((aumx::k_xdt_tm_fwd<false, 2, NW, NC>), grid, block, 0, s, g);
}
template <int NW> static void xdt_launch(const AumXdtArgs& g, hipStream_t s) {
    if (g.ncols == XDT_COLS) xdt_launch_nc<NW, XDT_COLS>(g, s);
    else xdt_launch_nc<NW, XDT_COLS_SMALL>(g, s);
}

extern "C" int aum_xdt_tm_fwd(const AumXdtArgs* p, void* stream) {
    const int rc = aumx::xdt_check(p);
    if (rc != AUM_OK) return rc;
    const AumXdtArgs& g = *p;
    const int ncu = cu_count();
    if (ncu <= 0) return AUM_E_LAUNCH;
    hipStream_t s = static_cast<hipStream_t>(stream);
    (void)hipGetLastError();
    switch (aumx::xdt_waves(g.ntok, ncu)) {
        case 8: xdt_launch<8>(g, s); break;
        case 9: xdt_launch<9>(g, s); break;
        case 10: xdt_launch<10>(g, s); break;
        case 11: xdt_launch<11>(g, s); break;
        default: xdt_launch<12>(g, s); break;
    }
    return hipGetLastError() == hipSuccess ? AUM_OK : AUM_E_LAUNCH;
}

template <int NW> static void xdt_bwd_launch(const AumXdtBwdArgs& g, hipStream_t s) {
    const dim3 grid((unsigned)((g.ntok + NW * XDT_TOK_W - 1) / (NW * XDT_TOK_W))), block(NW * 64);
    const bool bf = g.dtype == AUM_BF16, deep = g.dim % 512 == 0;
    if (bf && deep) hipLaunchKernelGGL((aumx::k_xdt_tm_bwd<true, 3, NW, 4>), grid, block, 0, s, g);
    else if (bf) hipLaunchKernelGGL((aumx::k_xdt_tm_bwd<true, 3, NW, 2>), grid, block, 0, s, g);
    else if (deep) hipLaunchKernelGGL((aumx::k_xdt_tm_bwd<false, 3, NW, 4>), grid, block, 0, s, g);
    else hipLaunchKernelGGL((aumx::k_xdt_tm_bwd<false, 3, NW, 2>), grid, block, 0, s, g);
}

extern "C" int aum_xdt_tm_bwd(const AumXdtBwdArgs* p, void* stream) {
    const int rc = aumx::xdt_bwd_check(p);
    if (rc != AUM_OK) return rc;
    const AumXdtBwdArgs& g = *p;
    const int ncu = cu_count();
    if (ncu <= 0) return AUM_E_LAUNCH;
    hipStream_t s = static_cast<hipStream_t>(stream);
    (void)hipGetLastError();
    switch (aumx::xdt_waves(g.ntok, ncu)) {
        case 8: xdt_bwd_launch<8>(g, s); break;
        case 9: xdt_bwd_launch<9>(g, s); break;
        case 10: xdt_bwd_launch<10>(g, s); break;
        case 11: xdt_bwd_launch<11>(g, s); break;
        default: xdt_bwd_launch<12>(g, s); break;
    }
    return hipGetLastError() == hipSuccess ? AUM_OK : AUM_E_LAUNCH;
}

extern "C" int aum_causal_conv1d_update(const AumConvUpdateArgs* p, void* stream) {
    const int rc = aumdec::conv_update_check(p);
    if (rc != AUM_OK) return rc;
    const int64_t n = (int64_t)p->batch * p->dim;
    const dim3 grid((unsigned)((n + 255) / 256)), block(256);
    hipStream_t s = static_cast<hipStream_t>(stream);
// ... 34 lines not shown
```

audio-mamba-aum_amd/csrc/scan_tm_kernels.h:

```cpp
#pragma once
#include "scan_kernels.h"

namespace aum {

#ifndef AUM_SCANT_ABL
#define AUM_SCANT_ABL 0
#endif
#ifndef AUM_SCANT_FWD_PAIRS
#define AUM_SCANT_FWD_PAIRS 1
#endif
constexpr int SCANT_N = 16;
constexpr int SCANT_CK = AUM_SCAN_TM_CK;
constexpr int SCANT_G = SCANT_CK / 2;
AUM_HOSTDEV constexpr int scant_nblocks(int len) { return (len + SCANT_CK - 1) / SCANT_CK; }
AUM_HOSTDEV constexpr int scant_nck(int len) { return scant_nblocks(len + SCANT_CK - 1) - 1; }
#ifdef AUM_SCANT_CK_F32
template <class T> AUM_HOSTDEV constexpr int scant_ck_rows() { return SCANT_N; }
#else
template <class T> AUM_HOSTDEV constexpr int scant_ck_rows() { return sizeof(T) == 2 ? SCANT_N / 2 : SCANT_N; }
#endif
AUM_HOSTDEV bool scant_supported(int dim, int dstate) { return dstate == SCANT_N && dim % WAVE == 0; }

template <bool V> struct ScanTTag { static constexpr bool value = V; };
template <class T> struct ScanTTile {
// ... 518 lines not shown
            if (PHASE >= 3) {
                AUM_UNROLL
                for (int j = 0; j < N / 2; ++j) P[AUM_W(w)][j] = spl2(splat(1.f));
                if (PHASE == 3)
                    scant_fwd_run<T, N, 3, SP, HAS_Z, HAS_PRE>(p, b, e0, d, rev ? L - 1 : 0, rev ? -1 : 1, it0, it1, Aptr, 1.f, x[AUM_W(w)], lw, nullptr,
                                                               P[AUM_W(w)]);
                else
                    scant_fwd_run<T, N, 4, SP, HAS_Z, HAS_PRE>(p, b, e0, d, rev ? 0 : L - 1, rev ? 1 : -1, L - it1, L - it0, Aptr, 1.f, x[AUM_W(w)], lw,
                                                               nullptr, P[AUM_W(w)]);
                float* cs = cb + (int64_t)s * (2 * N) * p.dim;
                AUM_UNROLL
                for (int n = 0; n < N; ++n) {
                    gstore(cs + (int64_t)n * p.dim, ec, (n & 1) ? hi2(P[AUM_W(w)][n >> 1]) : lo2(P[AUM_W(w)][n >> 1]), ec >= 0);
                    gstore(cs + (int64_t)(N + n) * p.dim, ec, (n & 1) ? hi2(x[AUM_W(w)][n >> 1]) : lo2(x[AUM_W(w)][n >> 1]), ec >= 0);
                }
            } else {
                for (int sp = 0; sp < s; ++sp) {
                    const float* cs = cb + (int64_t)sp * (2 * N) * p.dim;
                    AUM_UNROLL
                    for (int j = 0; j < N / 2; ++j) {
                        const vf2 pj = mk2(gload_u(cs + (int64_t)(2 * j) * p.dim, ec), gload_u(cs + (int64_t)(2 * j + 1) * p.dim, ec));
                        const vf2 xj = mk2(gload_u(cs + (int64_t)(N + 2 * j) * p.dim, ec), gload_u(cs + (int64_t)(N + 2 * j + 1) * p.dim, ec));
                        x[AUM_W(w)][j] = vfma2(pj, x[AUM_W(w)][j], xj);
                    }
                }
                scant_fwd_run<T, N, PHASE, SP, HAS_Z, HAS_PRE>(p, b, e0, d, rev ? L - 1 : 0, rev ? -1 : 1, it0, it1, Aptr, bidir ? 2.f : 1.f,
                                                               x[AUM_W(w)], lw);
            }
        }
    }
}

template <class T> AUM_HOSTDEV constexpr int scant_bwd_lds_wave_floats() {
    return 9 * ScanTTile<T>::FLOATS + 2 * SCANT_BC_BLOCK + 2 * SCANT_N * WAVE + 2 * ScanTTile<T>::NLD * WAVE + (sizeof(T) == 4 ? SCANT_BC_BLOCK : 0);
}
#ifndef AUM_SCANT_DBC_MERGE
#if defined(AUM_SCANT_CK_F32)
#define AUM_SCANT_DBC_MERGE 0
#else
#define AUM_SCANT_DBC_MERGE 1
#endif
#endif
AUM_HOSTDEV constexpr int scant_dbc_rows_to_sum(int nparts, bool bidir) { return bidir && AUM_SCANT_DBC_MERGE ? nparts / 2 : nparts; }
struct ScanTBwdOut {
    float* dbc;
    float* dA;
    float* dD;
    float* dbias;
    int nparts;
    float* carry;
    unsigned long long* trace;
};

#ifndef AUM_SCANT_TAIL2
#define AUM_SCANT_TAIL2 1
#endif
#ifndef AUM_SCANT_BABL
#define AUM_SCANT_BABL 0
#endif
template <class T, int N, int PHASE, bool SP, bool HAS_Z>
AUM_DEV void scant_bwd_run(const AumScanTmBwdArgs& p, const ScanTBwdOut& wo, int b, int e0, int dir, int part, int t0, int tstep, int it0,
                           int it1, const float* Aptr, float dmul, vf16& hh, vf16& dAacc, vf& dDacc, vf& dbacc, float* lds,
                           unsigned long long* tacc = nullptr) {
    using TL = ScanTTile<T>;
    constexpr int ES = TL::ES, NLD = TL::NLD;
    constexpr int LROW = 128, PLANE = SCANT_CK * LROW;
    constexpr bool FINAL = PHASE != 1, LD_PART = PHASE == 2;
    static_assert(N == 16 && SCANT_CK == 8, "8 steps x 8 state pairs");
    const int L = p.len;
    const vi lane = lane_id();
    const vi ec = lane + e0;
    const vf biasv = p.delta_bias ? gload_u(p.delta_bias, ec) : splat(0.f);
    const vf Dv = p.D ? gload_u(p.D, ec) * dmul : splat(0.f);
    const gbuf<T> ubuf = make_gbuf(row_ptr<T>(p.u, (int64_t)b * p.u_bs));
    const gbuf<T> dbuf = make_gbuf(row_ptr<T>(p.delta, (int64_t)b * p.delta_bs));
    const gbuf<T> zbuf = make_gbuf(HAS_Z ? row_ptr<T>(p.z, (int64_t)b * p.z_bs) : row_ptr<T>(p.u, 0));
    const gbuf<T> gbuf_ = make_gbuf(row_ptr<T>(p.dout, (int64_t)b * p.dout_bs));
    const gbuf<T> ybuf = make_gbuf(HAS_Z ? row_ptr<T>(p.out_pre, (int64_t)b * p.pre_bs) : row_ptr<T>(p.u, 0));
    const gbuf<T> dubuf = make_gbuf(row_ptr<T>(p.du, (int64_t)b * p.du_bs));
    const gbuf<T> ddbuf = make_gbuf(row_ptr<T>(p.ddelta, (int64_t)b * p.ddelta_bs));
    const gbuf<T> dzbuf = make_gbuf(HAS_Z ? row_ptr<T>(p.dz, (int64_t)b * p.dz_bs) : row_ptr<T>(p.du, 0));
    const gbuf<T> Bbuf = make_gbuf(row_ptr<T>(p.B, (int64_t)b * p.B_bs));
    const gbuf<T> Cbuf = make_gbuf(row_ptr<T>(p.C, (int64_t)b * p.C_bs));
    const gbuf<float> Abuf = make_gbuf(Aptr);
    const int nck = scant_nck(L);
    constexpr int CKR = scant_ck_rows<T>();
    constexpr int RPP = CKR / (N / 2);
    const gbuf<float> ckbuf = make_gbuf(p.ckpt + ((int64_t)dir * p.batch + b) * (nck > 0 ? nck : 1) * CKR * p.dim);
    const gbuf<float> dbcbuf = make_gbuf(wo.dbc + (int64_t)b * L * wo.nparts * (2 * N));
    const int u_tb = (int)p.u_ts * ES, d_tb = (int)p.delta_ts * ES, z_tb = HAS_Z ? (int)p.z_ts * ES : 0, g_tb = (int)p.dout_ts * ES,
              y_tb = HAS_Z ? (int)p.pre_ts * ES : 0, du_tb = (int)p.du_ts * ES, dd_tb = (int)p.ddelta_ts * ES,
              dz_tb = HAS_Z ? (int)p.dz_ts * ES : 0, B_tb = (int)p.B_ts * ES, C_tb = (int)p.C_ts * ES;
    constexpr bool DBC_MERGE = AUM_SCANT_DBC_MERGE && PHASE != 0;
    const int dbc_tb = wo.nparts * (2 * N) * 4;
    const int dbc_col_in = (wo.nparts / 2 + part) * (2 * N) * 4;
    const int dbc_col = DBC_MERGE && PHASE == 1 ? dbc_col_in : part * (2 * N) * 4;
    auto tok = [&](int it) { return t0 + it * tstep; };
    float* t_u0 = lds;
    float* t_d = lds + TL::FLOATS;
    float* t_z = lds + 2 * TL::FLOATS;
    float* t_g = lds + 3 * TL::FLOATS;
    float* t_y = lds + 4 * TL::FLOATS;
    float* t_du = lds + 5 * TL::FLOATS;
    float* t_dd = lds + 6 * TL::FLOATS;
    float* t_dz = lds + 7 * TL::FLOATS;
    float* t_bc = lds + 8 * TL::FLOATS;
    float* t_dbc = t_bc + SCANT_BC_BLOCK;
    float* t_u1 = t_dbc + SCANT_BC_BLOCK;
    float* t_ck = t_u1 + TL::FLOATS;
    float* t_A = t_ck + N * WAVE;
    float* t_rawB = t_A + N * WAVE;
    float* t_rawC = t_rawB + NLD * WAVE;
    float* t_dbi = sizeof(T) == 4 ? t_rawC + NLD * WAVE : t_ck + CKR * WAVE;
// ... 82 lines not shown
    constexpr int RBN = ((HAS_Z ? 5 : 3) + 2) * NLD;
    constexpr int PART = LD_PART ? 2 * NLD + (DBC_MERGE ? 1 : 0) : 0;
    AUM_TMB_STAMP(0);
#ifndef AUM_SCANT_BPRIO
#define AUM_SCANT_BPRIO 1
#endif
#ifndef AUM_SCANT_BPRIO_SHIFT
#define AUM_SCANT_BPRIO_SHIFT 0
#endif
#ifndef AUM_SCANT_BPRIO_HI
#define AUM_SCANT_BPRIO_HI 3
#endif
    const int bslot = AUM_SCANT_BPRIO ? wave_slot_on_simd() : 0;
    auto do_block = [&](auto full_tag, int blk) {
        constexpr bool FULL = decltype(full_tag)::value;
        if (AUM_SCANT_BPRIO == 1) {
            if (((blk >> AUM_SCANT_BPRIO_SHIFT) + bslot) & 1) AUM_SET_PRIO(AUM_SCANT_BPRIO_HI);
            else AUM_SET_PRIO(0);
        } else if (AUM_SCANT_BPRIO == 2) {
            if (bslot & 1) AUM_SET_PRIO(1);
        }
        const int base = blk * SCANT_CK;
        const int s_lo = FULL ? 0 : (it0 > base ? it0 - base : 0);
        const int s_hi = FULL ? SCANT_CK : (it1 < base + SCANT_CK ? it1 - base : SCANT_CK);
        const int s_min = FULL || PHASE == 1 ? 0 : s_lo;
        const bool more = blk > blk_lo;
        const bool cknext = more && blk - 1 > 0;
        if (blk == blk_hi - 1) AUM_WAIT_VM(0);
        else if (blk > 0) AUM_WAIT_VM(PART + CKR + NST);
        else AUM_WAIT_VM(PART + NST);
        wave_lds_fence();
        AUM_TMB_STAMP(9);
        convert_bc();
        vf2 Pd[SCANT_CK / 2], Pu[SCANT_CK / 2], Q[SCANT_CK / 2];
        float* const t_u = t_u_of(blk);
        {
            vi ru[SCANT_CK], rd[SCANT_CK], rg[SCANT_CK], rz[SCANT_CK], ry[SCANT_CK];
            AUM_UNROLL
            for (int s = 0; s < SCANT_CK; ++s) {
                const vi off = el_off + s * LROW;
                ru[s] = lds_read_raw<T>(t_u, off);
                rd[s] = lds_read_raw<T>(t_d, off);
                rg[s] = lds_read_raw<T>(t_g, off);
                if (HAS_Z) rz[s] = lds_read_raw<T>(t_z, off);
                if (HAS_Z && FINAL) ry[s] = lds_read_raw<T>(t_y, off);
            }
            AUM_SCHED_FENCE();
            const vf2 bias2 = spl2(biasv), one2 = spl2(splat(1.f));
            AUM_UNROLL
            for (int i = 0; i < SCANT_CK / 2; ++i) {
                const int s0 = 2 * i, s1 = 2 * i + 1;
                const vf2 us = mk2(raw_to_f32<T>(ru[s0]), raw_to_f32<T>(ru[s1]));
                vf2 d = mk2(raw_to_f32<T>(rd[s0]), raw_to_f32<T>(rd[s1])) + bias2;
                if (SP) d = vsoftplus2(d);
                Pd[i] = d;
                Pu[i] = d * us;
                const vf2 go = mk2(raw_to_f32<T>(rg[s0]), raw_to_f32<T>(rg[s1]));
                if (HAS_Z) {
                    const vf2 zz = mk2(raw_to_f32<T>(rz[s0]), raw_to_f32<T>(rz[s1]));
                    const vf2 sg = vsigmoid2(zz);
                    Q[i] = go * (zz * sg);
                    if (FINAL) {
                        const vf2 yt = mk2(raw_to_f32<T>(ry[s0]), raw_to_f32<T>(ry[s1]));
                        const vf2 dzv = go * yt * (sg * vfma2(zz, one2 - sg, one2));
                        lds_write_elem<T>(t_dz, el_off + s0 * LROW, lo2(dzv));
                        lds_write_elem<T>(t_dz, el_off + s1 * LROW, hi2(dzv));
                    }
                } else {
                    Q[i] = go;
                }
            }
        }
        auto DS = [&](int s) { return (s & 1) ? bc_hi(Pd[s >> 1]) : bc_lo(Pd[s >> 1]); };
        auto US = [&](int s) { return (s & 1) ? bc_hi(Pu[s >> 1]) : bc_lo(Pu[s >> 1]); };
        AUM_TMB_STAMP(10);
        vf2 S1[SCANT_CK], S2[SCANT_CK];
        AUM_UNROLL
        for (int s = 0; s < SCANT_CK; ++s) S1[s] = S2[s] = spl2(splat(0.f));
        wave_lds_fence();
        const Rows rc = rows_of(blk);
        if (!(AUM_SCANT_BABL & 8)) {
            if (more) request_block(blk - 1, rows_of(blk - 1));
            if (LD_PART) {
                load_tile(dubuf, du_tb, rc, t_du);
                load_tile(ddbuf, dd_tb, rc, t_dd);
                if constexpr (DBC_MERGE)
                    gbuf_load16_lds(dbcbuf, rc.rowt * dbc_tb + st_c * 16 + dbc_col_in, rc.t_lo * dbc_tb, t_dbi);
            }
        }
        AUM_TMB_STAMP(1);
        _Pragma("nounroll")
        for (int j = 0; j < N / 2; ++j) {
            if (AUM_SCANT_BPRIO == 3) {
                if (((j >> AUM_SCANT_BPRIO_SHIFT) + bslot) & 1) AUM_SET_PRIO(AUM_SCANT_BPRIO_HI);
                else AUM_SET_PRIO(0);
            }
            if (blk != blk_hi - 1) {
                if (more && cknext) AUM_WAIT_VM((CKR - RPP) + NST + RBN + PART);
                else if (more) AUM_WAIT_VM(NST + RBN + PART);
                else AUM_WAIT_VM(NST + PART);
            }
            const vf2 Aj = mk2(lds_read(t_A, lane + (2 * j) * WAVE), lds_read(t_A, lane + (2 * j + 1) * WAVE));
            vf2 x;
            if constexpr (RPP == 2) {
                x = mk2(lds_read(t_ck, lane + (2 * j) * WAVE), lds_read(t_ck, lane + (2 * j + 1) * WAVE));
            } else {
                vf x_lo, x_hi;
// ... 72 lines not shown
            vf dBsum;
            if (AUM_SCANT_BABL & 1) {
                dBsum = pb[0] + pb[7];
                dCsum = hc[0];
            } else if (AUM_SCANT_TAIL2) {
                wave_sum16_head(pb, hb);
                wave_sum16_tail2(hc, hb, dCsum, dBsum);
            } else {
                dBsum = wave_sum16(pb);
            }
            const vi slot = dbc_slot + 2 * j;
            lds_write(t_dbc, slot, dBsum);
            lds_write(t_dbc, slot + N, dCsum);
            vf16_set(hh, 2 * jr, lo2(hj));
            vf16_set(hh, 2 * jr + 1, hi2(hj));
            vf16_set(dAacc, 2 * jr, lo2(dAj));
            vf16_set(dAacc, 2 * jr + 1, hi2(dAj));
            AUM_TMB_STAMP(6);
        }
        if (cknext) AUM_WAIT_VM(CKR);
        else AUM_WAIT_VM(0);
        wave_lds_fence();
        if (more && !cknext) request_entry(0, 0, CKR);
        vi rus[SCANT_CK], rpu[SCANT_CK], rpd[SCANT_CK];
        AUM_UNROLL
        for (int s = 0; s < SCANT_CK; ++s) {
            const vi off = el_off + s * LROW;
            rus[s] = lds_read_raw<T>(t_u, off);
            if (FINAL && LD_PART) {
                rpu[s] = lds_read_raw<T>(t_du, off);
                rpd[s] = lds_read_raw<T>(t_dd, off);
            }
        }
        AUM_SCHED_FENCE();
        if constexpr (FULL) {
            const vf2 Dv2 = spl2(Dv), one2 = spl2(splat(1.f));
            AUM_UNROLL
            for (int i = 0; i < SCANT_CK / 2; ++i) {
                const int s0 = 2 * i, s1 = 2 * i + 1;
                const vf2 dls = Pd[i], dys = Q[i];
                const vf2 us = mk2(raw_to_f32<T>(rus[s0]), raw_to_f32<T>(rus[s1]));
                const vf2 s1v = mk2(lo2(S1[s0]) + hi2(S1[s0]), lo2(S1[s1]) + hi2(S1[s1]));
                const vf2 s2v = mk2(lo2(S2[s0]) + hi2(S2[s0]), lo2(S2[s1]) + hi2(S2[s1]));
                vf2 du = dls * s1v;
                vf2 dd = vfma2(us, s1v, s2v * spl2(splat(LN2)));
                if (FINAL) {
                    du = vfma2(Dv2, dys, du);
                    dDacc = vfma(lo2(dys), lo2(us), dDacc);
                    dDacc = vfma(hi2(dys), hi2(us), dDacc);
                    if (LD_PART) {
                        du = du + mk2(raw_to_f32<T>(rpu[s0]), raw_to_f32<T>(rpu[s1]));
                        dd = dd + mk2(raw_to_f32<T>(rpd[s0]), raw_to_f32<T>(rpd[s1]));
                    }
                    if (SP) dd = dd * (one2 - vexp2_2(dls * spl2(splat(-LOG2E))));
                    dbacc = dbacc + lo2(dd);
                    dbacc = dbacc + hi2(dd);
                }
                lds_write_elem<T>(t_du, el_off + s0 * LROW, lo2(du));
                lds_write_elem<T>(t_du, el_off + s1 * LROW, hi2(du));
                lds_write_elem<T>(t_dd, el_off + s0 * LROW, lo2(dd));
                lds_write_elem<T>(t_dd, el_off + s1 * LROW, hi2(dd));
            }
        } else {
            AUM_UNROLL
            for (int s = 0; s < SCANT_CK; ++s) {
                if (s >= s_lo && s < s_hi) {
                    const vi off = el_off + s * LROW;
                    const vf dls = (s & 1) ? hi2(Pd[s >> 1]) : lo2(Pd[s >> 1]), dys = (s & 1) ? hi2(Q[s >> 1]) : lo2(Q[s >> 1]);
                    const vf us = raw_to_f32<T>(rus[s]);
                    const vf s1 = lo2(S1[s]) + hi2(S1[s]), s2 = lo2(S2[s]) + hi2(S2[s]);
                    vf du = dls * s1;
                    vf dd = vfma(us, s1, s2 * LN2);
                    if (FINAL) {
                        du = vfma(Dv, dys, du);
                        dDacc = vfma(dys, us, dDacc);
                        if (LD_PART) {
                            du = du + raw_to_f32<T>(rpu[s]);
                            dd = dd + raw_to_f32<T>(rpd[s]);
                        }
                        if (SP) dd = dd * (splat(1.f) - vexp2(dls * (-LOG2E)));
                        dbacc = dbacc + dd;
                    }
                    lds_write_elem<T>(t_du, off, du);
                    lds_write_elem<T>(t_dd, off, dd);
                }
            }
        }
        wave_lds_fence();
        AUM_TMB_STAMP(7);
        store_tile(dubuf, du_tb, t_du, rc);
        store_tile(ddbuf, dd_tb, t_dd, rc);
        if (HAS_Z && FINAL) store_tile(dzbuf, dz_tb, t_dz, rc);
        {
            vq q = lds_read16(t_dbc, st_i * (SCANT_BC_ROW * 4) + st_c * 16);
            if constexpr (DBC_MERGE && LD_PART) {
                const vq qi = lds_read16(t_dbi, st_i * (SCANT_BC_ROW * 4) + st_c * 16);
                AUM_UNROLL
                for (int k = 0; k < 4; ++k) q.w[k] = f32_as_int(int_as_f32(q.w[k]) + int_as_f32(qi.w[k]));
            }
            if (rc.inside) gbuf_store16(dbcbuf, rc.rowt * dbc_tb + st_c * 16 + dbc_col, rc.t_lo * dbc_tb, q);
            else gbuf_store16_m(dbcbuf, rc.rowt * dbc_tb + st_c * 16 + dbc_col, 0, q, rc.valid);
        }
        wave_lds_fence();
        AUM_TMB_STAMP(8);
    };
    for (int blk = blk_hi - 1; blk >= blk_lo; --blk) {
        if (blk * SCANT_CK >= it0 && blk * SCANT_CK + SCANT_CK <= it1) do_block(ScanTTag<true>{}, blk);
        else do_block(ScanTTag<false>{}, blk);
    }
#undef AUM_TMB_STAMP
}

template <class T, bool SP, bool HAS_Z, bool BIDIR>
AUM_DEV void scant_bwd(const AumScanTmBwdArgs& p, const ScanTBwdOut& wo, int wg, float* lds, unsigned long long* tacc = nullptr) {
    constexpr int N = SCANT_N;
    constexpr int NW = SCANT_NW;
    constexpr int UPW = scant_units_per_wg<BIDIR>();
    const int gpb = p.dim / WAVE;
    const int units = p.batch * gpb;
    const int L = p.len;
    vf16 hh[AUM_PER_WAVE(NW)], dA[AUM_PER_WAVE(NW)];
    vf dD[AUM_PER_WAVE(NW)], dbias[AUM_PER_WAVE(NW)];
    auto finish = [&](int w, int unit, int d) {
        const int b = unit / gpb, e0 = (unit % gpb) * WAVE;
        const vi ec = lane_id() + e0;
        float* pa = wo.dA + ((int64_t)d * p.batch + b) * N * p.dim;
        AUM_UNROLL
        for (int n = 0; n < N; ++n) gstore(pa + (int64_t)n * p.dim, ec, vf16_get(dA[AUM_W(w)], n), ec >= 0);
        gstore(wo.dD + ((int64_t)d * p.batch + b) * p.dim, ec, dD[AUM_W(w)] * (BIDIR ? 2.f : 1.f), ec >= 0);
        gstore(wo.dbias + ((int64_t)d * p.batch + b) * p.dim, ec, dbias[AUM_W(w)], ec >= 0);
    };
    auto init = [&](int w) {
        AUM_UNROLL
        for (int n = 0; n < N; ++n) {
            vf16_set(hh[AUM_W(w)], n, splat(0.f));
            vf16_set(dA[AUM_W(w)], n, splat(0.f));
        }
        dD[AUM_W(w)] = dbias[AUM_W(w)] = splat(0.f);
    };
    if (!BIDIR) {
        const bool rev = (p.flags & AUM_SCAN_REVERSE) != 0;
        AUM_FOR_EACH_WAVE(w, NW) {
            const int unit = wg * UPW + w;
            if (unit < units) {
                init(w);
                scant_bwd_run<T, N, 0, SP, HAS_Z>(p, wo, unit / gpb, (unit % gpb) * WAVE, 0, unit % gpb, rev ? L - 1 : 0, rev ? -1 : 1, 0, L, p.A, 1.f,
                                                  hh[AUM_W(w)], dA[AUM_W(w)], dD[AUM_W(w)], dbias[AUM_W(w)], lds + w * scant_bwd_lds_wave_floats<T>(), tacc);
                finish(w, unit, 0);
            }
        }
        return;
    }
    const int npairs = units;
    _Pragma("nounroll")
    for (int stage = 0; stage < 3; ++stage) {
        AUM_FOR_EACH_WAVE(w, NW) {
            const int h = w >> 1, d = w & 1, io = scant_grid_shift(L, d);
            const int slot = h == 0 ? (stage == 2 ? 1 : 0) : (stage == 0 ? 1 : 2);
            const int phase = h == 0 ? (stage == 0 ? 1 : 2) : (stage == 2 ? 2 : 1);
            const int unit = wg * 3 + slot;
            if (unit < npairs) {
                const int b = unit / gpb, e0 = (unit % gpb) * WAVE, prt = AUM_SCANT_DBC_MERGE ? unit % gpb : (unit % gpb) * 2 + d;
                float* cy = wo.carry + ((int64_t)wg * 2 + d) * (2 * N + 2) * WAVE;
                const vi lane = lane_id();
                if (phase == 1) {
                    init(w);
                    scant_bwd_run<T, N, 1, SP, HAS_Z>(p, wo, b, e0, d, prt, d ? L - 1 + io : -io, d ? -1 : 1, scant_first_half(L, d) + io, L + io, d ? p.A_b : p.A, 2.f,
                                                      hh[AUM_W(w)], dA[AUM_W(w)], dD[AUM_W(w)], dbias[AUM_W(w)],
                                                      lds + w * scant_bwd_lds_wave_floats<T>(), tacc);
                    if (slot == 1) {
                        AUM_UNROLL
                        for (int n = 0; n < N; ++n) {
                            gstore(cy + n * WAVE, lane, vf16_get(hh[AUM_W(w)], n), lane >= 0);
                            gstore(cy + (N + n) * WAVE, lane, vf16_get(dA[AUM_W(w)], n), lane >= 0);
                        }
                        gstore(cy + 2 * N * WAVE, lane, dD[AUM_W(w)], lane >= 0);
                        gstore(cy + (2 * N + 1) * WAVE, lane, dbias[AUM_W(w)], lane >= 0);
                    }
                } else {
                    if (slot == 1) {
                        AUM_UNROLL
                        for (int n = 0; n < N; ++n) {
                            vf16_set(hh[AUM_W(w)], n, gload_u(cy + n * WAVE, lane));
                            vf16_set(dA[AUM_W(w)], n, gload_u(cy + (N + n) * WAVE, lane));
                        }
                        dD[AUM_W(w)] = gload_u(cy + 2 * N * WAVE, lane);
                        dbias[AUM_W(w)] = gload_u(cy + (2 * N + 1) * WAVE, lane);
                    }
                    scant_bwd_run<T, N, 2, SP, HAS_Z>(p, wo, b, e0, d, prt, d ? L - 1 + io : -io, d ? -1 : 1, io, scant_first_half(L, d) + io, d ? p.A_b : p.A, 2.f,
                                                      hh[AUM_W(w)], dA[AUM_W(w)], dD[AUM_W(w)], dbias[AUM_W(w)],
                                                      lds + w * scant_bwd_lds_wave_floats<T>(), tacc);
                    finish(w, unit, d);
                }
            }
        }
        if (stage < 2) AUM_WG_BARRIER();
    }
}

template <class T, int PHASE, bool SP, bool HAS_Z>
AUM_DEV void scant_seg_bwd(const AumScanTmBwdArgs& p, const ScanTBwdOut& wo, const ScanTSeg& sg, int wg, float* lds) {
    constexpr int N = SCANT_N;
    constexpr int NW = SCANT_NW;
    const int gpb = p.dim / WAVE;
    const int L = p.len;
    const int items = p.batch * gpb * sg.nseg;
    const bool bidir = p.A_b != nullptr;
    vf16 hh[AUM_PER_WAVE(NW)], dA[AUM_PER_WAVE(NW)];
    vf dD[AUM_PER_WAVE(NW)], dbias[AUM_PER_WAVE(NW)];
    AUM_FOR_EACH_WAVE(w, NW) {
        const int item = wg * NW + w;
        if (item < items) {
            const int d = sg.dir0, s = item % sg.nseg, unit = item / sg.nseg;
            const int b = unit / gpb, e0 = (unit % gpb) * WAVE, prt = bidir && !AUM_SCANT_DBC_MERGE ? (unit % gpb) * 2 + d : unit % gpb;
            const bool rev = bidir ? d == 1 : (p.flags & AUM_SCAN_REVERSE) != 0;
            const int it0 = s * sg.seg_len < L ? s * sg.seg_len : L;
            const int it1 = it0 + sg.seg_len < L ? it0 + sg.seg_len : L;
            const vi ec = lane_id() + e0;
            AUM_UNROLL
            for (int n = 0; n < N; ++n) {
                vf16_set(hh[AUM_W(w)], n, splat(0.f));
                vf16_set(dA[AUM_W(w)], n, splat(0.f));
            }
            dD[AUM_W(w)] = dbias[AUM_W(w)] = splat(0.f);
            const float* cb = sg.carry + ((int64_t)d * p.batch + b) * sg.nseg * (2 * N) * p.dim;
            for (int sp = sg.nseg - 1; sp > s; --sp) {
                const float* cs = cb + (int64_t)sp * (2 * N) * p.dim;
                AUM_UNROLL
                for (int n = 0; n < N; ++n)
                    vf16_set(hh[AUM_W(w)], n, vfma(gload_u(cs + (int64_t)n * p.dim, ec), vf16_get(hh[AUM_W(w)], n), gload_u(cs + (int64_t)(N + n) * p.dim, ec)));
            }
            scant_bwd_run<T, N, PHASE, SP, HAS_Z>(p, wo, b, e0, d, prt, rev ? L - 1 : 0, rev ? -1 : 1, it0, it1, d ? p.A_b : p.A, bidir ? 2.f : 1.f,
                                                  hh[AUM_W(w)], dA[AUM_W(w)], dD[AUM_W(w)], dbias[AUM_W(w)], lds + w * scant_bwd_lds_wave_floats<T>());
            const int64_t q = ((int64_t)d * p.batch + b) * sg.nseg + s;
            float* pa = wo.dA + q * N * p.dim;
            AUM_UNROLL
            for (int n = 0; n < N; ++n) gstore(pa + (int64_t)n * p.dim, ec, vf16_get(dA[AUM_W(w)], n), ec >= 0);
            gstore(wo.dD + q * p.dim, ec, dD[AUM_W(w)] * (bidir ? 2.f : 1.f), ec >= 0);
            gstore(wo.dbias + q * p.dim, ec, dbias[AUM_W(w)], ec >= 0);
        }
    }
}

}
```

audio-mamba-aum_amd/csrc/xdt_args.h:

```cpp
#pragma once
#include <stdint.h>

#include "../../include/aum_hip.h"

#define XDT_COLS 80
#define XDT_COLS_SMALL 56
#ifndef XDT_TOK_W
#define XDT_TOK_W 16
#endif
#define XDT_WAVES_MIN 8
#define XDT_WAVES_MAX 12
#define XDT_MAX_DIM 1536

namespace aumx {
inline int xdt_check(const AumXdtArgs* p) {
    if (!p || !p->u || !p->wx || !p->wdt || !p->x_dbl || !p->delta) return AUM_E_NULL;
    const AumXdtArgs& g = *p;
    if (g.ntok <= 0 || g.dim <= 0 || g.rank <= 0 || g.ncols <= 0 || g.ldu < g.dim || g.ldwx < g.dim || g.ldwdt < g.rank || g.ldx < g.ncols ||
        g.ldd < g.dim)
        return AUM_E_SHAPE;
    if (g.dtype != AUM_BF16 && g.dtype != AUM_F16) return AUM_E_DTYPE;
    if ((g.ncols != XDT_COLS && g.ncols != XDT_COLS_SMALL) || g.rank % 8 || g.rank > 64 || g.rank > g.ncols || g.dim % 256 || g.dim > XDT_MAX_DIM) return AUM_E_UNSUPPORTED;
    if (g.ldu % 8 || g.ldwx % 8 || g.ldwdt % 8 || g.ldx % 8 || g.ldd % 8) return AUM_E_UNSUPPORTED;
    if (((uintptr_t)g.u | (uintptr_t)g.wx | (uintptr_t)g.wdt | (uintptr_t)g.x_dbl | (uintptr_t)g.delta) & 15u) return AUM_E_UNSUPPORTED;
    return AUM_OK;
}
inline int xdt_bwd_check(const AumXdtBwdArgs* p) {
    if (!p || !p->ddelta || !p->dbc || !p->wdt_t || !p->wx_t || !p->du || !p->dx_dbl) return AUM_E_NULL;
    const AumXdtBwdArgs& g = *p;
    if (g.ntok <= 0 || g.dim <= 0 || g.rank <= 0 || g.ncols <= 0 || g.ldd < g.dim || g.ldu < g.dim || g.ldwdt < g.dim || g.ldwx < g.ncols ||
        g.ldx < g.ncols || g.lddbc < g.ncols - g.rank)
        return AUM_E_SHAPE;
    if (g.dtype != AUM_BF16 && g.dtype != AUM_F16) return AUM_E_DTYPE;
    if (g.ncols != XDT_COLS || g.rank != XDT_COLS - 32 || g.dim % 256 || g.dim > XDT_MAX_DIM) return AUM_E_UNSUPPORTED;
    if (g.ldd % 8 || g.ldu % 8 || g.ldwdt % 8 || g.ldwx % 8 || g.ldx % 8 || g.lddbc % 4) return AUM_E_UNSUPPORTED;
    if (((uintptr_t)g.ddelta | (uintptr_t)g.dbc | (uintptr_t)g.wdt_t | (uintptr_t)g.wx_t | (uintptr_t)g.du | (uintptr_t)g.dx_dbl) & 15u)
        return AUM_E_UNSUPPORTED;
    return AUM_OK;
}
inline int xdt_waves(int64_t ntok, int ncu) {
    const int64_t frags = (ntok + XDT_TOK_W - 1) / XDT_TOK_W;
    int best = XDT_WAVES_MIN;
    int64_t best_cost = -1;
    for (int nw = XDT_WAVES_MIN; nw <= XDT_WAVES_MAX; ++nw) {
        const int64_t wgs = (frags + nw - 1) / nw, cost = (wgs + ncu - 1) / ncu * nw;
        if (best_cost < 0 || cost < best_cost) {
            best = nw;
            best_cost = cost;
        }
    }
    return best;
}
}
```

audio-mamba-aum_amd/csrc/xdt_kernels.h:

```cpp
#pragma once
#include <hip/hip_runtime.h>
#include <stdint.h>

#include "xdt_args.h"

namespace aumx {

typedef __bf16 bf8v __attribute__((ext_vector_type(8)));
typedef _Float16 h8v __attribute__((ext_vector_type(8)));
typedef short s8v __attribute__((ext_vector_type(8)));
typedef float f4v __attribute__((ext_vector_type(4)));
typedef float f2v __attribute__((ext_vector_type(2)));
typedef __bf16 bf2v __attribute__((ext_vector_type(2)));
typedef _Float16 h2v __attribute__((ext_vector_type(2)));
typedef uint32_t u4v __attribute__((ext_vector_type(4)));
typedef uint32_t u2v __attribute__((ext_vector_type(2)));

template <bool BF16> __device__ __forceinline__ f4v mfma(s8v a, s8v b, f4v c) {
    if constexpr (BF16) return __builtin_amdgcn_mfma_f32_16x16x32_bf16(__builtin_bit_cast(bf8v, a), __builtin_bit_cast(bf8v, b), c, 0, 0, 0);
    else return __builtin_amdgcn_mfma_f32_16x16x32_f16(__builtin_bit_cast(h8v, a), __builtin_bit_cast(h8v, b), c, 0, 0, 0);
}
template <bool BF16> __device__ __forceinline__ uint32_t pack2(float a, float b) {
    if constexpr (BF16) return __builtin_bit_cast(uint32_t, __builtin_convertvector(f2v{a, b}, bf2v));
    else return __builtin_bit_cast(uint32_t, __builtin_convertvector(f2v{a, b}, h2v));
}

template <bool BF16> __device__ __forceinline__ float lo16(uint32_t v) {
    if constexpr (BF16) return __builtin_bit_cast(float, v << 16);
    else return (float)__builtin_bit_cast(h2v, v)[0];
}
template <bool BF16> __device__ __forceinline__ float hi16(uint32_t v) {
    if constexpr (BF16) return __builtin_bit_cast(float, v & 0xffff0000u);
    else return (float)__builtin_bit_cast(h2v, v)[1];
}

constexpr int NCF = XDT_COLS / 16;
constexpr int NTF = XDT_TOK_W / 16;
constexpr int XP = XDT_COLS * 2 + 16;
constexpr int XT_BYTES = XDT_TOK_W * XP;
constexpr int WDP = 144;
__host__ __device__ constexpr int slab_pitch(int kh) { return kh * 2 + 16; }
__host__ __device__ constexpr int slab_bytes(int dim) {
    const int a = XDT_COLS * slab_pitch(dim / 2), b = (dim / 2) * WDP;
    return a > b ? a : b;
}
__host__ __device__ constexpr int lds_bytes(int dim, int nw) { return slab_bytes(dim) + nw * XT_BYTES; }

template <int NT>
__device__ __forceinline__ void stage_rows(char* dst, int dst_pitch, const char* src, int64_t src_pitch, int rows, int chunks, int tid) {
    const int total = rows * chunks;
    for (int base = tid; base < total; base += NT * 8) {
        u4v r[8];
#pragma unroll
        for (int j = 0; j < 8; ++j) {
            const int idx = base + j * NT;
            if (idx < total) {
                const int row = idx / chunks, ch = idx - row * chunks;
                r[j] = *reinterpret_cast<const u4v*>(src + row * src_pitch + ch * 16);
            }
        }
#pragma unroll
        for (int j = 0; j < 8; ++j) {
            const int idx = base + j * NT;
            if (idx < total) {
                const int row = idx / chunks, ch = idx - row * chunks;
                *reinterpret_cast<u4v*>(dst + row * dst_pitch + ch * 16) = r[j];
            }
        }
    }
}

template <bool BF16, int KS, int NW, int NC>
__global__ __launch_bounds__(NW * 64, 1) void k_xdt_tm_fwd(AumXdtArgs g) {
    constexpr int NCF = (NC + 15) / 16;
    constexpr int XP = NC == 80 ? 176 : 144;
    static_assert(NC % 8 == 0 && NCF * 32 <= XP && XP <= aumx::XP, "tile row holds every fragment column");
    __shared__ __attribute__((aligned(16))) char lds[lds_bytes(XDT_MAX_DIM, NW)];
    const int tid = (int)threadIdx.x, lane = tid & 63, w = tid >> 6;
    const int rho = lane & 15, kg = lane >> 4;
    const int E = g.dim, KH = E / 2, SP = slab_pitch(KH);
    char* slab = lds;
    char* xt = lds + slab_bytes(E) + w * XT_BYTES;
    const int64_t t0 = (int64_t)blockIdx.x * (NW * XDT_TOK_W) + w * XDT_TOK_W;
    const s8v zero = {0, 0, 0, 0, 0, 0, 0, 0};
    const char* ub = static_cast<const char*>(g.u);
    bool tok_ok[NTF];
    const char* urow[NTF];
    for (int tf = 0; tf < NTF; ++tf) {
        tok_ok[tf] = t0 + tf * 16 + rho < g.ntok;
        urow[tf] = ub + ((t0 + tf * 16 + rho) * g.ldu + kg * 16) * 2;
    }

    f4v acc[NTF][NCF];
#pragma unroll
    for (int tf = 0; tf < NTF; ++tf)
#pragma unroll
        for (int f = 0; f < NCF; ++f) acc[tf][f] = f4v{0.f, 0.f, 0.f, 0.f};

    auto load_u = [&](int k0, s8v (&uf)[NTF][2]) {
#pragma unroll
        for (int tf = 0; tf < NTF; ++tf) {
            uf[tf][0] = tok_ok[tf] ? *reinterpret_cast<const s8v*>(urow[tf] + (int64_t)k0 * 2) : zero;
            uf[tf][1] = tok_ok[tf] ? *reinterpret_cast<const s8v*>(urow[tf] + (int64_t)k0 * 2 + 16) : zero;
        }
    };
    const int nsteps = KH / 64, total = E / 64;
    s8v ur[4][NTF][2];
#pragma unroll
    for (int j = 0; j < 4; ++j)
        if (j < total) load_u(j * 64, ur[j]);
    const char* wrd = slab + rho * SP + kg * 32;
    for (int s0 = 0; s0 < total; s0 += 4) {
#pragma unroll
        for (int j = 0; j < 4; ++j) {
            const int s = s0 + j;
            if (s == 0 || s == nsteps) {
                __syncthreads();
                stage_rows<NW * 64>(slab, SP, static_cast<const char*>(g.wx) + (int64_t)(s / nsteps) * KH * 2, (int64_t)g.ldwx * 2, NC, KH / 8, tid);
                __syncthreads();
            }
            const int sl = s >= nsteps ? s - nsteps : s;
#pragma unroll
            for (int f = 0; f < NCF; ++f) {
                const s8v w0 = *reinterpret_cast<const s8v*>(wrd + f * 16 * SP + sl * 128);
                const s8v w1 = *reinterpret_cast<const s8v*>(wrd + f * 16 * SP + sl * 128 + 16);
#pragma unroll
                for (int tf = 0; tf < NTF; ++tf) {
                    acc[tf][f] = mfma<BF16>(w0, ur[j][tf][0], acc[tf][f]);
                    acc[tf][f] = mfma<BF16>(w1, ur[j][tf][1], acc[tf][f]);
                }
            }
            if (s + 4 < total) load_u((s + 4) * 64, ur[j]);
        }
    }
#pragma unroll
    for (int tf = 0; tf < NTF; ++tf)
#pragma unroll
        for (int f = 0; f < NCF; ++f) {
            u2v v;
            v.x = pack2<BF16>(acc[tf][f][0], acc[tf][f][1]);
            v.y = pack2<BF16>(acc[tf][f][2], acc[tf][f][3]);
            *reinterpret_cast<u2v*>(xt + (tf * 16 + rho) * XP + (f * 16 + kg * 4) * 2) = v;
        }
    __builtin_amdgcn_s_waitcnt(0xc07f);
    {
        char* xo = static_cast<char*>(g.x_dbl);
        constexpr int PIECES = NC * 2 / 16;
        for (int idx = lane; idx < XDT_TOK_W * PIECES; idx += 64) {
            const int tk = idx / PIECES, pc = idx - tk * PIECES;
            if (t0 + tk < g.ntok)
                *reinterpret_cast<u4v*>(xo + ((t0 + tk) * g.ldx) * 2 + pc * 16) = *reinterpret_cast<const u4v*>(xt + tk * XP + pc * 16);
        }
    }
    s8v xf[NTF][KS];
#pragma unroll
    for (int tf = 0; tf < NTF; ++tf)
#pragma unroll
        for (int ks = 0; ks < KS; ++ks) {
            const int k = ks * 32 + kg * 8;
            xf[tf][ks] = k < g.rank ? *reinterpret_cast<const s8v*>(xt + (tf * 16 + rho) * XP + k * 2) : zero;
        }
    const bool k_ok[2] = {kg * 8 < g.rank, 32 + kg * 8 < g.rank};
    const int CH = E / 2, wchunks = g.rank / 8;
    char* ob = static_cast<char*>(g.delta) + ((t0 + rho) * g.ldd + kg * 8) * 2;
    const int64_t otf = (int64_t)16 * g.ldd * 2;
    const char* wdr = slab + ((rho >> 2) * 8 + (rho & 3)) * WDP + kg * 16;
    for (int half = 0; half < 2; ++half) {
        __syncthreads();
        stage_rows<NW * 64>(slab, WDP, static_cast<const char*>(g.wdt) + (int64_t)half * CH * g.ldwdt * 2, (int64_t)g.ldwdt * 2, CH, wchunks, tid);
        __syncthreads();
        const int npairs = CH / 32;
#pragma unroll 2
        for (int p = 0; p < npairs; ++p) {
            s8v wf[2][KS];
#pragma unroll
            for (int j = 0; j < 2; ++j)
#pragma unroll
                for (int ks = 0; ks < KS; ++ks)
                    wf[j][ks] = k_ok[ks] ? *reinterpret_cast<const s8v*>(wdr + (p * 32 + j * 4) * WDP + ks * 64) : zero;
#pragma unroll
            for (int tf = 0; tf < NTF; ++tf) {
                f4v a2[2] = {f4v{0.f, 0.f, 0.f, 0.f}, f4v{0.f, 0.f, 0.f, 0.f}};
#pragma unroll
                for (int j = 0; j < 2; ++j)
#pragma unroll
                    for (int ks = 0; ks < KS; ++ks) a2[j] = mfma<BF16>(wf[j][ks], xf[tf][ks], a2[j]);
                if (tok_ok[tf]) {
                    u4v o;
                    o.x = pack2<BF16>(a2[0][0], a2[0][1]);
                    o.y = pack2<BF16>(a2[0][2], a2[0][3]);
                    o.z = pack2<BF16>(a2[1][0], a2[1][1]);
                    o.w = pack2<BF16>(a2[1][2], a2[1][3]);
                    *reinterpret_cast<u4v*>(ob + tf * otf + ((int64_t)half * CH + p * 32) * 2) = o;
                }
            }
        }
    }
}

constexpr int WXP = 256;

template <bool BF16, int RF, int NW, int PD>
__global__ __launch_bounds__(NW * 64, 1) void k_xdt_tm_bwd(AumXdtBwdArgs g) {
    __shared__ __attribute__((aligned(16))) char lds[lds_bytes(XDT_MAX_DIM, NW)];
    constexpr int R = RF * 16, KS = 3;
    const int tid = (int)threadIdx.x, lane = tid & 63, w = tid >> 6;
    const int rho = lane & 15, kg = lane >> 4;
    const int E = g.dim, KH = E / 2, SP = slab_pitch(KH);
    char* slab = lds;
    char* xt = lds + slab_bytes(XDT_MAX_DIM) + w * XT_BYTES;
    const int64_t t0 = (int64_t)blockIdx.x * (NW * XDT_TOK_W) + w * XDT_TOK_W;
    const s8v zero = {0, 0, 0, 0, 0, 0, 0, 0};
    const bool tok_ok = t0 + rho < g.ntok;
    const char* drow = static_cast<const char*>(g.ddelta) + ((t0 + rho) * g.ldd + kg * 16) * 2;

    f4v acc[RF];
#pragma unroll
    for (int f = 0; f < RF; ++f) acc[f] = f4v{0.f, 0.f, 0.f, 0.f};
    auto load_d = [&](int k0, s8v (&df)[2]) {
        df[0] = tok_ok ? *reinterpret_cast<const s8v*>(drow + (int64_t)k0 * 2) : zero;
        df[1] = tok_ok ? *reinterpret_cast<const s8v*>(drow + (int64_t)k0 * 2 + 16) : zero;
    };
    const int nsteps = KH / 64, total = E / 64;
    s8v dr[4][2];
#pragma unroll
    for (int j = 0; j < 4; ++j)
        if (j < total) load_d(j * 64, dr[j]);
    const char* wrd = slab + rho * SP + kg * 32;
    for (int s0 = 0; s0 < total; s0 += 4) {
#pragma unroll
        for (int j = 0; j < 4; ++j) {
            const int s = s0 + j;
            if (s == 0 || s == nsteps) {
                __syncthreads();
                stage_rows<NW * 64>(slab, SP, static_cast<const char*>(g.wdt_t) + (int64_t)(s / nsteps) * KH * 2, (int64_t)g.ldwdt * 2, R, KH / 8, tid);
                __syncthreads();
            }
            const int sl = s >= nsteps ? s - nsteps : s;
#pragma unroll
            for (int f = 0; f < RF; ++f) {
                const s8v w0 = *reinterpret_cast<const s8v*>(wrd + f * 16 * SP + sl * 128);
                const s8v w1 = *reinterpret_cast<const s8v*>(wrd + f * 16 * SP + sl * 128 + 16);
                acc[f] = mfma<BF16>(w0, dr[j][0], acc[f]);
                acc[f] = mfma<BF16>(w1, dr[j][1], acc[f]);
            }
// ... 112 lines not shown
```

audio-mamba-aum_amd/mamba_ssm/ops/selective_scan_interface.py:

```python
import contextlib
import os

import torch
import torch.nn.functional as F

import aum_hip

_DBG = os.environ.get("AUM_DEBUG") == "1"


def _dbg_env(name, default):
    return os.environ.get(name, default) if _DBG else default


_STEP_CACHE_ON = _dbg_env("AUM_STEP_CACHE", "1") != "0"
_WGRAD_SPLIT_ON = _dbg_env("AUM_WGRAD_SPLIT", "1") != "0"
_REF_DZ_DROP = os.environ.get("AUM_REF_DZ_DROP", "0") == "1"
TOKEN_MAJOR = _dbg_env("AUM_TOKEN_MAJOR", "1") != "0"

_custom_fwd = torch.amp.custom_fwd(device_type="cuda")
_custom_bwd = torch.amp.custom_bwd(device_type="cuda")


def _autocast_dtype():
# ... 338 lines not shown
        return torch.matmul(a, b)
    out = torch.empty((ntok, b.shape[1]), dtype=a.dtype, device=a.device)
    torch.matmul(a[:n0], b, out=out[:n0])
    torch.matmul(a[n0:], b, out=out[n0:])
    return out


_V2_STREAMS = _dbg_env("AUM_V2_STREAMS", "1") != "0"
_side_streams = {}
_main_streams = {}
def v2_two_streams(params=(), module=None):
    if not _V2_STREAMS:
        return False
    import torch.distributed as dist
    if dist.is_available() and dist.is_initialized() and not getattr(module, "_aum_streams_joined", False):
        return False
    return not any(getattr(p_, "_post_accumulate_grad_hooks", None) for p_ in params)


def side_streams(device):
    s = _side_streams.get(device)
    if s is None:
        s = _side_streams[device] = (torch.cuda.Stream(device=device), torch.cuda.Stream(device=device))
    _main_streams[device] = torch.cuda.current_stream(device)
    return s


def ddp_join_streams_hook(hook=None):
    from torch.distributed.algorithms.ddp_comm_hooks import default_hooks
    inner = hook or default_hooks.allreduce_hook

    def joined(state, bucket):
        buf = bucket.buffer()
        if buf.is_cuda:
            cur = torch.cuda.current_stream(buf.device)
            for s in tuple(_side_streams.get(buf.device) or ()) + (_main_streams.get(buf.device),):
                if s is not None and s != cur:
                    cur.wait_stream(s)
        return inner(state, bucket)

    return joined


def register_ddp_join_streams(ddp, state=None, hook=None):
    ddp.register_comm_hook(state, ddp_join_streams_hook(hook))
    for m in ddp.module.modules():
        if getattr(m, "bimamba_type", None) == "v2":
            m._aum_streams_joined = True


_XDT_BWD_HIP = _dbg_env("AUM_XDT_BWD_LIB", "0") != "1"
_XDT_HIP = _dbg_env("AUM_XDT_LIB", "0") != "1"
_DTPROJ_HIP = _dbg_env("AUM_DTPROJ_LIB", "0") != "1"
_GEMM_MODE = _dbg_env("AUM_GEMM", "auto")
if _GEMM_MODE not in ("auto", "hip", "lib"):
    raise ValueError("AUM_GEMM takes auto, hip or lib")
_HIP_GEMM = _GEMM_MODE != "lib"
_HIP_GEMM_FASTER = {(1536, 768), (3072, 768)}
if _dbg_env("AUM_GEMM_SHAPES", ""):
    _HIP_GEMM_FASTER = {tuple(int(v) for v in sh.split("x")) for sh in _dbg_env("AUM_GEMM_SHAPES", "").replace("+", ",").split(",")}


def _hip_gemm_ok(a, n, k):
    return (_HIP_GEMM and a.is_cuda and a.dtype in (torch.bfloat16, torch.float16) and n % aum_hip.GEMM_BN == 0 and k % aum_hip.GEMM_BK == 0
            and (_GEMM_MODE == "hip" or (n, k) in _HIP_GEMM_FASTER))


def _gemm_rows(a, w_nk, bit):
    if _hip_gemm_ok(a, w_nk.shape[0], w_nk.shape[1]) and aum_hip.gemm_tn_supported(a, w_nk):
        return aum_hip.gemm_tn(a, w_nk)
    return _mm_rows(a, w_nk.t(), bit)


def _weight_t_for_dgrad(w_param, w_cast, a_is_cuda):
    n, k = w_cast.shape[1], w_cast.shape[0]
    if not (_HIP_GEMM and a_is_cuda and w_cast.dtype in (torch.bfloat16, torch.float16) and n % aum_hip.GEMM_BN == 0 and k % aum_hip.GEMM_BK == 0
            and (_GEMM_MODE == "hip" or (n, k) in _HIP_GEMM_FASTER)):
        return None
    return _cast_t(w_param, w_cast.dtype)


def _gemm_dgrad(g, w_cast, w_t, bit):
    if w_t is not None and aum_hip.gemm_tn_supported(g, w_t):
        return aum_hip.gemm_tn(g, w_t)
    return _mm_rows(g, w_cast, bit)


class InProjTmFn(torch.autograd.Function):

    @staticmethod
    def forward(ctx, weight, hidden2d):
        w = _cast(weight, _autocast_dtype())
        h = hidden2d.to(w.dtype)
        w_t = _weight_t_for_dgrad(weight, w, h.is_cuda) if ctx.needs_input_grad[1] else None
        ctx.save_for_backward(w, h, w_t)
        ctx.wdtype, ctx.hdtype = weight.dtype, hidden2d.dtype
        ctx.wparam = weight
        return _gemm_rows(h, w, 1)

    @staticmethod
    def backward(ctx, dxz2d):
        w, h, w_t = ctx.saved_tensors
        dxz2d = dxz2d.to(w.dtype)
        dh = _gemm_dgrad(dxz2d, w, w_t, 8) if ctx.needs_input_grad[1] else None
        home = grad_home(ctx.wparam)
        dw = _homed(_wgrad_tm(dxz2d, h, _WGRAD_SPLITS[0], ctx.wdtype, home=home), home) if ctx.needs_input_grad[0] else None
# ... 25 lines not shown
def token_major_ok(d_inner, d_state, d_conv, dt_rank, dtype=None):
    es = 2 if dtype in (torch.bfloat16, torch.float16) else 4
    return (aum_hip.scan_tm_supported(d_inner, d_state) and d_conv <= 4 and (dt_rank * es) % 16 == 0
            and ((dt_rank + 2 * d_state) * es) % 16 == 0)


_TM_MIN_WAVES = int(_dbg_env("AUM_TM_MIN_WAVES", "1536"))


_TM_SEGMENTS = int(_dbg_env("AUM_TM_SEGMENTS", "-1"))


def tm_segments(batch, d_inner, seqlen, bidirectional, training, device=None):
    if _TM_SEGMENTS == 0 or seqlen is None:
        return 1
    if _TM_SEGMENTS > 1:
        return min(_TM_SEGMENTS, aum_hip.SCAN_TM_MAX_SEGMENTS)
    return aum_hip.scan_tm_segments(batch, d_inner, seqlen, bidirectional, training, device=device)


def token_major_preferred(batch, d_inner, bidirectional, training=None, seqlen=None):
    training = torch.is_grad_enabled() if training is None else training
    need = -(-_TM_MIN_WAVES * 4 // 3) if training and bidirectional else _TM_MIN_WAVES
    if batch * (d_inner // 64) * (2 if bidirectional else 1) >= need:
        return True
    return tm_segments(batch, d_inner, seqlen, bidirectional, training) > 1


def _is_tm(xz):
    return xz.dim() == 3 and xz.stride(1) == 1 and xz.shape[1] > 1


def _inner_forward_tm(ctx, xz, conv1d_weight, conv1d_bias, x_proj_weight, delta_proj_weight, out_proj_weight, out_proj_bias, A, A_b, D,
                      delta_bias, delta_softplus, reverse):
    act = _autocast_dtype()
    ctx.out_proj_wdtype = out_proj_weight.dtype if out_proj_weight is not None else None
    x_proj_param, delta_proj_param = x_proj_weight, delta_proj_weight
    x_proj_weight, delta_proj_weight = _cast(x_proj_weight, act), _cast(delta_proj_weight, act)
    out_proj_param = out_proj_weight
    out_proj_weight, out_proj_bias = _cast(out_proj_weight, act), _cast(out_proj_bias, act)
    out_proj_wt = None
    if out_proj_weight is not None and any(ctx.needs_input_grad):
        out_proj_wt = _weight_t_for_dgrad(out_proj_param, out_proj_weight.to(xz.dtype), xz.is_cuda)
    xz_t = xz.transpose(1, 2)
    Bsz, L, two_e = xz_t.shape
    E = two_e // 2
    R = delta_proj_weight.shape[1]
    N = A.shape[-1]
    x, z = xz_t[:, :, :E], xz_t[:, :, E:]
    conv_w = conv1d_weight.reshape(E, -1)
    conv_out = aum_hip.conv1d_tm_fwd(x, conv_w, conv1d_bias, True, reverse)
    conv2d = conv_out.view(Bsz * L, E)
    w_x, w_dt = x_proj_weight.to(conv2d.dtype), delta_proj_weight.to(conv2d.dtype)
    if _XDT_HIP and conv2d.is_cuda and aum_hip.xdt_tm_supported(conv2d, w_x, w_dt):
        x_dbl, delta = aum_hip.xdt_tm_fwd(conv2d, w_x, w_dt)
    else:
        x_dbl = torch.matmul(conv2d, w_x.t())
        delta = None
    if delta is not None:
        pass
    elif _DTPROJ_HIP and x_dbl.is_cuda and aum_hip.dtproj_tm_supported(x_dbl, R, w_dt):
        delta = aum_hip.dtproj_tm_fwd(x_dbl, R, w_dt)
    else:
        delta = torch.matmul(x_dbl[:, :R], w_dt.t())
    x3 = x_dbl.view(Bsz, L, R + 2 * N)
    Bm, Cm = x3[:, :, R:R + N], x3[:, :, R + N:]
    need_bwd = any(ctx.needs_input_grad)
    w_x_t = w_dt_t = None
    if need_bwd and _XDT_BWD_HIP and conv2d.is_cuda and R + 2 * N == aum_hip.XDT_COLS and R == aum_hip.XDT_COLS - 32 and E % 256 == 0 \
            and E <= aum_hip.XDT_MAX_DIM and conv2d.dtype in (torch.bfloat16, torch.float16):
        w_x_t, w_dt_t = _cast_t(x_proj_param, conv2d.dtype), _cast_t(delta_proj_param, conv2d.dtype)
    ckpt = aum_hip.scan_tm_ckpt(Bsz, L, E, N, A_b is not None, xz.device, dtype=conv_out.dtype) if need_bwd else None
    waves = Bsz * (E // 64) * (2 if A_b is not None else 1)
    cut = waves < (-(-_TM_MIN_WAVES * 4 // 3) if need_bwd and A_b is not None else _TM_MIN_WAVES)
    out_z, out_pre = aum_hip.scan_tm_fwd(conv_out, delta.view(Bsz, L, E), A, Bm, Cm, D, z, delta_bias, delta_softplus,
                                         reverse if A_b is None else False, A_b=A_b, want_out_pre=need_bwd, ckpt=ckpt,
                                         segments=tm_segments(Bsz, E, L, A_b is not None, False, device=xz.device) if cut else 1)
    ctx.tm_cut = cut
    ctx.A_cached = (need_bwd and A.dtype == torch.float32 and A.is_contiguous() and A.data_ptr() in _A_CACHE_PTRS
                    and (A_b is None or (A_b.is_contiguous() and A_b.data_ptr() in _A_CACHE_PTRS)))
    ctx.tm = True
    ctx.params = dict(conv_w=conv1d_weight, conv_b=conv1d_bias, x_proj=x_proj_param, dt_proj=delta_proj_param, out_proj=out_proj_param, D=D,
                      dt_bias=delta_bias, A_log=_A_OWNER.get(A.data_ptr()), A_b_log=None if A_b is None else _A_OWNER.get(A_b.data_ptr()))
    ctx.delta_softplus, ctx.reverse = delta_softplus, reverse
    ctx.has_out_proj = out_proj_weight is not None
    ctx.out_proj_bias_is_None = out_proj_bias is None
    ctx.save_for_backward(xz, conv_w, conv1d_bias, x_dbl, x_proj_weight, delta_proj_weight, out_proj_weight, conv_out, delta, A, A_b, D,
                          delta_bias, out_pre, out_z, ckpt, out_proj_wt, w_x_t, w_dt_t)
    if out_proj_weight is None:
        return out_z.transpose(1, 2)
    out = _gemm_rows(out_z.view(Bsz * L, E), out_proj_weight.to(out_z.dtype), 2)
    if out_proj_bias is not None:
        out = out + out_proj_bias
    return out.reshape(Bsz, L, -1)


def _inner_backward_tm(ctx, dout):
    (xz, conv_w, conv1d_bias, x_dbl, x_proj_weight, delta_proj_weight, out_proj_weight, conv_out, delta, A, A_b, D, delta_bias, out_pre,
     out_z, ckpt, out_proj_wt, w_x_t, w_dt_t) = ctx.saved_tensors
    xz_t = xz.transpose(1, 2)
    Bsz, L, two_e = xz_t.shape
    E = two_e // 2
    R = delta_proj_weight.shape[1]
    N = A.shape[-1]
    x, z = xz_t[:, :, :E], xz_t[:, :, E:]
    dxz_t = torch.empty((Bsz, L, two_e), dtype=xz.dtype, device=xz.device)
    dx, dz = dxz_t[:, :, :E], dxz_t[:, :, E:]
    dout_proj_weight = dout_proj_bias = None
    pend = _PendingSums()
    H = {k: grad_home(v) for k, v in getattr(ctx, "params", {}).items()}
    H = {k: H.get(k) for k in ("conv_w", "conv_b", "x_proj", "dt_proj", "out_proj", "D", "dt_bias", "A_log", "A_b_log")}
    if ctx.has_out_proj:
        dout2 = dout.reshape(Bsz * L, -1).to(out_proj_weight.dtype)
        dout_z = _gemm_dgrad(dout2, out_proj_weight, out_proj_wt, 4).view(Bsz, L, E).to(conv_out.dtype)
        dout_proj_weight = _wgrad_tm(dout2, out_z.view(Bsz * L, E), _WGRAD_SPLITS[1], ctx.out_proj_wdtype, pend, home=H["out_proj"])
        dout_proj_bias = dout2.sum(0) if not ctx.out_proj_bias_is_None else None
    else:
        dout_z = dout.transpose(1, 2)
        dout_z = (dout_z if dout_z.stride(2) == 1 else dout_z.contiguous()).to(xz.dtype)
    x3 = x_dbl.view(Bsz, L, R + 2 * N)
    g = aum_hip.scan_tm_bwd(conv_out, delta.view(Bsz, L, E), A, x3[:, :, R:R + N], x3[:, :, R + N:], D, z, delta_bias, dout_z, out_pre,
                            ckpt, ctx.delta_softplus, ctx.reverse if A_b is None else False, A_b=A_b, dz_out=dz,
                            segments=tm_segments(Bsz, E, L, A_b is not None, True, device=conv_out.device) if ctx.tm_cut else 1,
                            want_dA_xA=ctx.A_cached,
                            param_out=dict(dD=H["D"], ddelta_bias=H["dt_bias"], dA_xA=H["A_log"], dA_b_xA=H["A_b_log"]))
    if ctx.A_cached:
        _da_xa_put(g["dA"], g["dA_xA"], A)
        if A_b is not None:
            _da_xa_put(g["dA_b"], g["dA_b_xA"], A_b)
    du2, ddelta2 = g["du"].view(Bsz * L, E), g["ddelta"].view(Bsz * L, E)
    dbc2 = g["dBC"].view(Bsz * L, 2 * N)
    conv2d = conv_out.view(Bsz * L, E)
    if w_x_t is not None and aum_hip.xdt_tm_bwd_supported(ddelta2, dbc2, w_dt_t, w_x_t, du2):
        dx_dbl = aum_hip.xdt_tm_bwd(ddelta2, dbc2, w_dt_t, w_x_t, du2)
        splits = _pick_splits(Bsz * L, _WGRAD_SPLITS[1])
        if aum_hip.gemm_wgrad_supported(ddelta2, x_dbl[:, :R]) and aum_hip.gemm_wgrad_supported(conv2d, dx_dbl):
            ddelta_proj_weight = pend.add(aum_hip.gemm_wgrad(ddelta2, x_dbl[:, :R], partials=True), out=H["dt_proj"])
            dx_proj_weight = pend.add(aum_hip.gemm_wgrad(conv2d, dx_dbl, partials=True), R + 2 * N, out=H["x_proj"])
        else:
            ddelta_proj_weight = split_k_wgrad(ddelta2.t(), x_dbl[:, :R], splits, torch.float32)
            dx_proj_weight = split_k_wgrad(dx_dbl.t(), conv2d, splits, torch.float32)
    else:
        dx_dbl = torch.empty_like(x_dbl)
        dx_dbl[:, R:].copy_(dbc2)
        dx_dbl[:, :R].copy_(torch.matmul(ddelta2, delta_proj_weight.to(ddelta2.dtype)))
        splits = _pick_splits(Bsz * L, _WGRAD_SPLITS[1])
        ddelta_proj_weight = split_k_wgrad(ddelta2.t(), x_dbl[:, :R], splits, torch.float32)
        dx_proj_weight = split_k_wgrad(dx_dbl.t(), conv2d, splits, torch.float32)
        du2.addmm_(dx_dbl, x_proj_weight.to(dx_dbl.dtype))
    _, dconv_w, dconv_b = aum_hip.conv1d_tm_bwd(x, conv_w, conv1d_bias, g["du"], True, ctx.reverse, dx_out=dx, partials=True)
    dconv_w, dconv_b = pend.add(dconv_w, out=H["conv_w"]), (None if dconv_b is None else pend.add(dconv_b, out=H["conv_b"]))
    sums = pend.run()
    dout_proj_weight, ddelta_proj_weight, dx_proj_weight, dconv_w, dconv_b = (
        sums[v] if isinstance(v, _PendingIndex) else v for v in (dout_proj_weight, ddelta_proj_weight, dx_proj_weight, dconv_w, dconv_b))
    return dict(dxz=dxz_t.transpose(1, 2), dconv_w=_homed(dconv_w.reshape(E, 1, -1), H["conv_w"]), dconv_b=_homed(dconv_b, H["conv_b"]),
                dx_proj_w=_homed(dx_proj_weight, H["x_proj"]), ddt_proj_w=_homed(ddelta_proj_weight, H["dt_proj"]),
                dout_proj_w=_homed(dout_proj_weight, H["out_proj"]), dout_proj_b=dout_proj_bias,
                dA=g["dA"], dA_b=g.get("dA_b"), dD=_homed(g["dD"], H["D"]), ddelta_bias=_homed(g["ddelta_bias"], H["dt_bias"]),
                dB_proj_bias=None, dC_proj_bias=None)


def _dm2d(t):
    Bsz, E, L = t.shape
    return t.permute(1, 0, 2).reshape(E, Bsz * L)


def _is_dmajor(t):
    Bsz, E, L = t.shape
    return t.stride(2) == 1 and t.stride(0) == L and t.stride(1) == Bsz * L


def _inner_forward(ctx, xz, conv1d_weight, conv1d_bias, x_proj_weight, delta_proj_weight, out_proj_weight,
                   out_proj_bias, A, A_b, D, delta_bias, B_proj_bias, C_proj_bias, delta_softplus, reverse):
    if A.is_complex():
        raise NotImplementedError("real A only (SSI:502 asserts the same for the bidirectional path)")
    ctx.tm = False
    if (TOKEN_MAJOR and not (_REF_DZ_DROP and A_b is not None) and _is_tm(xz) and B_proj_bias is None and C_proj_bias is None
# ... 283 lines not shown
```

include/aum_hip.h:

```cpp
#ifndef AUM_HIP_H
#define AUM_HIP_H

#include <stdint.h>

#ifdef __cplusplus
extern "C" {
#endif

#define AUM_ABI_VERSION 13

enum { AUM_F32 = 0, AUM_BF16 = 1, AUM_F16 = 2 };

enum {
    AUM_OK = 0,
    AUM_E_NULL = -1,
    AUM_E_SHAPE = -2,
    AUM_E_DTYPE = -3,
    AUM_E_UNSUPPORTED = -4,
    AUM_E_WORKSPACE = -5,
    AUM_E_LAUNCH = -6
};

#define AUM_SCAN_SOFTPLUS 1u
#define AUM_SCAN_REVERSE 2u
#define AUM_SCAN_GENERIC 4u
#define AUM_SCAN_ROWPAIR 8u
#define AUM_SCAN_ACCUMULATE 16u
#define AUM_CONV_SILU 1u
#define AUM_CONV_REVERSE 2u
#define AUM_CONV_GENERIC 4u
#define AUM_GEMM_LOCKSTEP 1u
#define AUM_GEMM_PIPELINED 32u
#define AUM_GEMM_PACED 256u
#define AUM_NORM_PRENORM 1u
#define AUM_NORM_GENERIC 2u

typedef struct AumScanFwdArgs {
    const void *u, *delta, *z, *B, *C;
    const float *A, *A_b, *D, *delta_bias;
    void *out, *out_pre;
    float *last_state;
    void *workspace;
    int64_t workspace_bytes;
    int64_t u_bs, u_ds;
    int64_t delta_bs, delta_ds;
    int64_t z_bs, z_ds;
    int64_t B_bs, B_ns;
    int64_t C_bs, C_ns;
    int64_t out_bs, out_ds;
    int32_t batch, dim, len, dstate;
    int32_t dtype;
    uint32_t flags;
    float *x_ck;
    float *x_lane;
} AumScanFwdArgs;

typedef struct AumScanBwdArgs {
    const void *u, *delta, *z, *B, *C, *dout, *out_pre;
    const float *A, *A_b, *D, *delta_bias;
    void *du, *ddelta, *dz;
    float *dA, *dA_b, *dB, *dC, *dD, *ddelta_bias;
    void *workspace;
    int64_t workspace_bytes;
    int64_t u_bs, u_ds, delta_bs, delta_ds, z_bs, z_ds, B_bs, B_ns, C_bs, C_ns;
    int64_t dout_bs, dout_ds, out_bs, out_ds;
    int64_t du_bs, du_ds, ddelta_bs, ddelta_ds, dz_bs, dz_ds;
    int64_t dB_bs, dB_ns, dC_bs, dC_ns;
    int32_t batch, dim, len, dstate;
    int32_t dtype;
    uint32_t flags;
    const float *x_ck;
    const float *x_lane;
} AumScanBwdArgs;

int aum_selective_scan_fwd(const AumScanFwdArgs* args, void* stream);
int aum_selective_scan_bwd(const AumScanBwdArgs* args, void* stream);
int aum_scan_max_single_pass_len(void);
int64_t aum_selective_scan_workspace_bytes(int32_t batch, int32_t dim, int32_t len, int32_t dstate, int32_t bidirectional,
                                           int32_t backward);
int64_t aum_selective_scan_ckpt_bytes(int32_t batch, int32_t dim, int32_t len, int32_t dstate);
// ... 128 lines not shown

typedef struct AumConvTmArgs {
    const void *x, *dy;
    const float *weight, *bias;
    void *y;
    void *dx;
    float *dw_part, *db_part;
    int64_t x_bs, x_ts, y_bs, y_ts, dy_bs, dy_ts, dx_bs, dx_ts;
    int32_t batch, dim, len, width;
    int32_t dtype;
    uint32_t flags;
} AumConvTmArgs;
int aum_conv1d_tm_fwd(const AumConvTmArgs* args, void* stream);
int aum_conv1d_tm_bwd(const AumConvTmArgs* args, void* stream);
int32_t aum_conv1d_tm_nparts(int32_t batch, int32_t len);

typedef struct AumGemmArgs {
    const void *a, *b;
    void *c;
    int32_t m, n, k;
    int32_t lda, ldb, ldc;
    int32_t dtype;
    uint32_t flags;
} AumGemmArgs;
int aum_gemm_tn(const AumGemmArgs* args, void* stream);

typedef struct AumGemmWArgs {
    const void *y, *x;
    float* part;
    int64_t t;
    int64_t ldy, ldx;
    int32_t n, k, splits;
    int32_t dtype;
} AumGemmWArgs;
int aum_gemm_wgrad(const AumGemmWArgs* args, void* stream);

typedef struct AumDtProjArgs {
    const void *x, *w;
    void *out;
    int64_t ntok;
    int32_t dim, rank;
    int32_t ldx, ldw, ldo;
    int32_t dtype;
} AumDtProjArgs;
int aum_dtproj_tm_fwd(const AumDtProjArgs* args, void* stream);

typedef struct AumXdtArgs {
    const void *u, *wx, *wdt;
    void *x_dbl, *delta;
    int64_t ntok;
    int32_t dim, rank, ncols;
    int32_t ldu, ldwx, ldwdt, ldx, ldd;
    int32_t dtype;
} AumXdtArgs;
int aum_xdt_tm_fwd(const AumXdtArgs* args, void* stream);

typedef struct AumXdtBwdArgs {
    const void *ddelta;
    const float *dbc;
    const void *wdt_t, *wx_t;
    void *du, *dx_dbl;
    int64_t ntok;
    int32_t dim, rank, ncols;
    int32_t ldd, lddbc, ldwdt, ldwx, ldu, ldx;
    int32_t dtype;
} AumXdtBwdArgs;
int aum_xdt_tm_bwd(const AumXdtBwdArgs* args, void* stream);

typedef struct AumConvUpdateArgs {
    const void* x;
    float* conv_state;
    const float *weight, *bias;
    void* out;
    int32_t batch, dim, width;
    int32_t dtype;
    uint32_t flags;
} AumConvUpdateArgs;
int aum_causal_conv1d_update(const AumConvUpdateArgs* args, void* stream);
typedef struct AumStateUpdateArgs {
    float* state;
    const void *x, *dt, *z, *B, *C;
    const float *A, *D, *dt_bias;
    void* out;
    int32_t batch, dim, dstate;
    int32_t dtype;
    uint32_t flags;
} AumStateUpdateArgs;
int aum_selective_state_update(const AumStateUpdateArgs* args, void* stream);

int aum_abi_version(void);
int aum_selftest_wave_scan(const float* in, float* out, int rev, void* stream);
int aum_selftest_wave_sum32(const float* in, float* out, void* stream);
int aum_hbm_copy(const void* src, void* dst, int64_t bytes, void* stream);

int aum_sum_rows(const void* src, float* dst, int64_t batch, int64_t outer, int64_t inner, int32_t src_dtype, void* stream);

#define AUM_SUM_MAX_JOBS 8
typedef struct AumSumJob {
    const float* src;
    float* dst;
    int64_t outer, inner;
    int32_t tr_cols;
    int32_t reserved;
} AumSumJob;
int aum_sum_rows_multi(const AumSumJob* jobs, int32_t njobs, void* stream);

int aum_cast_bank(const uint64_t* src, int32_t n, int32_t rows, int32_t cols, void* bank, void* bank_t, int32_t dtype, void* stream);
// ... 27 lines not shown
```

Baseline: 1069 clips/s.

## Fuse delta bias and softplus into xdt projection epilogue, skip in scan

```diff
diff --git a/audio-mamba-aum_amd/aum_hip/__init__.py b/audio-mamba-aum_amd/aum_hip/__init__.py
--- a/audio-mamba-aum_amd/aum_hip/__init__.py
+++ b/audio-mamba-aum_amd/aum_hip/__init__.py
@@ -9,6 +9,8 @@
 
 AUM_F32, AUM_BF16, AUM_F16 = 0, 1, 2
 SCAN_SOFTPLUS, SCAN_REVERSE, SCAN_GENERIC, SCAN_ROWPAIR, SCAN_ACCUMULATE = 1, 2, 4, 8, 16
+SCAN_DELTA_ACTIVATED = 32
+XDT_DELTA_SOFTPLUS = 1
 CONV_SILU, CONV_REVERSE = 1, 2
 _DT = {torch.float32: AUM_F32, torch.bfloat16: AUM_BF16, torch.float16: AUM_F16}
 _ERR = {-1: "AUM_E_NULL", -2: "AUM_E_SHAPE", -3: "AUM_E_DTYPE", -4: "AUM_E_UNSUPPORTED", -5: "AUM_E_WORKSPACE",
@@ -179,7 +181,8 @@
 
 class XdtArgs(C.Structure):
     _fields_ = ([(n, _vp) for n in ("u", "wx", "wdt", "x_dbl", "delta")] + [("ntok", _i64)]
-                + [(n, _i32) for n in ("dim", "rank", "ncols", "ldu", "ldwx", "ldwdt", "ldx", "ldd", "dtype")])
+                + [(n, _i32) for n in ("dim", "rank", "ncols", "ldu", "ldwx", "ldwdt", "ldx", "ldd", "dtype")]
+                + [("delta_bias", _vp), ("flags", _u32)])
 
 
 EXPORTS = ["aum_gemm_tn", "aum_dtproj_tm_fwd", "aum_xdt_tm_fwd", "aum_proj_fwd", "aum_proj_bwd_data", "aum_proj_bwd_weight", "aum_proj_bwd_weight_splits", "aum_fbank_fwd", "aum_frontend_tokens_fwd", "aum_abi_version", "aum_selective_scan_fwd", "aum_selective_scan_bwd", "aum_scan_max_single_pass_len",
@@ -538,7 +541,7 @@
 
 
 def scan_tm_fwd(u, delta, A, B, C, D=None, z=None, delta_bias=None, delta_softplus=False, reverse=False, A_b=None,
-                want_out_pre=False, ckpt=None, out=None, lib=None, segments=1):
+                want_out_pre=False, ckpt=None, out=None, lib=None, segments=1, delta_activated=False):
     lib = lib or get()
     batch, length, dim = u.shape
     dstate = A.shape[1]
@@ -572,7 +575,7 @@
         lib.check_tensor(ckpt)
         a.ckpt = _ptr(ckpt)
     a.batch, a.dim, a.len, a.dstate, a.dtype = batch, dim, length, dstate, _DT[u.dtype]
-    a.flags = (SCAN_SOFTPLUS if delta_softplus else 0) | (SCAN_REVERSE if reverse else 0)
+    a.flags = (SCAN_SOFTPLUS if delta_softplus else 0) | (SCAN_REVERSE if reverse else 0) | (SCAN_DELTA_ACTIVATED if delta_activated else 0)
     if segments > 1:
         sa = ScanTmSegFwdArgs()
         sa.base = a
@@ -591,7 +594,7 @@
 
 
 def scan_tm_bwd(u, delta, A, B, C, D, z, delta_bias, dout, out_pre, ckpt, delta_softplus=False, reverse=False, A_b=None, dz_out=None,
-                lib=None, segments=1, want_dA_xA=False, param_out=None):
+                lib=None, segments=1, want_dA_xA=False, param_out=None, delta_activated=False):
     lib = lib or get()
     batch, length, dim = u.shape
     dstate = A.shape[1]
@@ -655,7 +658,7 @@
         a.pre_bs, a.pre_ts = _tm3(out_pre, "out_pre", dim)
         a.dz_bs, a.dz_ts = _tm3(dz, "dz", dim)
     a.batch, a.dim, a.len, a.dstate, a.dtype = batch, dim, length, dstate, _DT[u.dtype]
-    a.flags = (SCAN_SOFTPLUS if delta_softplus else 0) | (SCAN_REVERSE if reverse else 0)
+    a.flags = (SCAN_SOFTPLUS if delta_softplus else 0) | (SCAN_REVERSE if reverse else 0) | (SCAN_DELTA_ACTIVATED if delta_activated else 0)
     if segments > 1:
         sa = ScanTmSegBwdArgs()
         sa.base = a
@@ -859,12 +862,21 @@
     return dx_dbl
 
 
-def xdt_tm_fwd(u, wx, wdt, lib=None):
+def xdt_tm_fwd(u, wx, wdt, lib=None, delta_bias=None, delta_softplus=False):
     lib = lib or get()
     for t in (u, wx, wdt):
         lib.check_tensor(t)
     if not xdt_tm_supported(u, wx, wdt):
         raise RuntimeError(f"xdt_tm_fwd: unsupported operands {tuple(u.shape)} {u.dtype}, {tuple(wx.shape)}, {tuple(wdt.shape)}")
+    if delta_bias is not None and not delta_softplus:
+        raise RuntimeError("xdt_tm_fwd: delta_bias is only added together with the softplus (delta_softplus=True)")
+    if delta_softplus and lib.host:
+        raise RuntimeError("xdt_tm_fwd: delta_softplus needs the device library")
+    if delta_bias is not None:
+        delta_bias = _f32c(delta_bias)
+        lib.check_tensor(delta_bias)
+        if delta_bias.shape != (u.shape[1],) or delta_bias.data_ptr() % 16:
+            raise RuntimeError(f"xdt_tm_fwd: delta_bias must be a 16-byte aligned ({u.shape[1]},) fp32 tensor")
     ntok, dim = u.shape
     rank = wdt.shape[1]
     ncols = wx.shape[0]
@@ -874,6 +886,7 @@
     a.u, a.wx, a.wdt, a.x_dbl, a.delta = _ptr(u), _ptr(wx), _ptr(wdt), _ptr(x_dbl), _ptr(delta)
     a.ntok, a.dim, a.rank, a.ncols = ntok, dim, rank, ncols
     a.ldu, a.ldwx, a.ldwdt, a.ldx, a.ldd, a.dtype = u.stride(0), wx.stride(0), wdt.stride(0), ncols, dim, _DT[u.dtype]
+    a.delta_bias, a.flags = _ptr(delta_bias), (XDT_DELTA_SOFTPLUS if delta_softplus else 0)
     _launch(lib.c.aum_xdt_tm_fwd, a, u, lib, "xdt_tm_fwd", (ntok, dim, rank))
     return x_dbl, delta
 
diff --git a/audio-mamba-aum_amd/csrc/aum_api_tm.inc b/audio-mamba-aum_amd/csrc/aum_api_tm.inc
--- a/audio-mamba-aum_amd/csrc/aum_api_tm.inc
+++ b/audio-mamba-aum_amd/csrc/aum_api_tm.inc
@@ -139,7 +139,7 @@
 #endif
 #if AUM_API_PART == 6 || AUM_API_PART == 0
 #ifndef AUM_EMU
-template <class T, bool SP, bool HAS_Z, bool BIDIR>
+template <class T, int SP, bool HAS_Z, bool BIDIR>
 __global__ __launch_bounds__(SCANT_NW * 64, AUM_SCANT_BWD_MINW) void k_scant_bwd(AumScanTmBwdArgs a, ScanTBwdOut wo) {
     __shared__ __attribute__((aligned(16))) float lds[SCANT_NW * scant_bwd_lds_wave_floats<T>()];
 #ifdef AUM_SCANT_TRACE
@@ -159,7 +159,7 @@
 #endif
 }
 #endif
-template <class T, bool SP, bool HAS_Z, bool BIDIR> static int launch_scant_bwd(const AumScanTmBwdArgs& a, const ScanTBwdOut& wo, aum_stream_t s) {
+template <class T, int SP, bool HAS_Z, bool BIDIR> static int launch_scant_bwd(const AumScanTmBwdArgs& a, const ScanTBwdOut& wo, aum_stream_t s) {
     const int grid = scant_bwd_wgs<BIDIR>(a.batch * (a.dim / WAVE));
 #ifdef AUM_EMU
     (void)s;
@@ -171,22 +171,27 @@
     return launch_status();
 }
 template <class T> static int scan_tm_bwd_t(const AumScanTmBwdArgs& a, const ScanTBwdOut& wo, aum_stream_t s) {
+    if (a.flags & AUM_SCAN_DELTA_ACTIVATED) {
+        if constexpr (sizeof(T) == 2)
+            return a.A_b ? launch_scant_bwd<T, SCANT_SP_ACT, true, true>(a, wo, s) : launch_scant_bwd<T, SCANT_SP_ACT, true, false>(a, wo, s);
+        return AUM_E_UNSUPPORTED;
+    }
     const int key = ((a.flags & AUM_SCAN_SOFTPLUS) ? 4 : 0) | (a.z ? 2 : 0) | (a.A_b ? 1 : 0);
     switch (key) {
-#define AUM_TMB(K) case K: return launch_scant_bwd<T, ((K) & 4) != 0, ((K) & 2) != 0, ((K) & 1) != 0>(a, wo, s);
+#define AUM_TMB(K) case K: return launch_scant_bwd<T, ((K) & 4) ? SCANT_SP_IN : SCANT_SP_NONE, ((K) & 2) != 0, ((K) & 1) != 0>(a, wo, s);
         AUM_TMB(0) AUM_TMB(1) AUM_TMB(2) AUM_TMB(3) AUM_TMB(4) AUM_TMB(5) AUM_TMB(6) AUM_TMB(7)
 #undef AUM_TMB
     }
     return AUM_E_UNSUPPORTED;
 }
 #ifndef AUM_EMU
-template <class T, int PHASE, bool SP, bool HAS_Z>
+template <class T, int PHASE, int SP, bool HAS_Z>
 __global__ __launch_bounds__(SCANT_NW * 64, AUM_SCANT_BWD_MINW) void k_scant_seg_bwd(AumScanTmBwdArgs a, ScanTBwdOut wo, ScanTSeg sg) {
     __shared__ __attribute__((aligned(16))) float lds[SCANT_NW * scant_bwd_lds_wave_floats<T>()];
     scant_seg_bwd<T, PHASE, SP, HAS_Z>(a, wo, sg, (int)blockIdx.x, lds);
 }
 #endif
-template <class T, int PHASE, bool SP, bool HAS_Z>
+template <class T, int PHASE, int SP, bool HAS_Z>
 static int launch_scant_seg_bwd(const AumScanTmBwdArgs& a, const ScanTBwdOut& wo, const ScanTSeg& sg, aum_stream_t s) {
     const int grid = (a.batch * (a.dim / WAVE) * sg.nseg + SCANT_NW - 1) / SCANT_NW;
 #ifdef AUM_EMU
@@ -199,9 +204,19 @@
     return launch_status();
 }
 template <class T> static int scan_tm_seg_bwd_t(const AumScanTmBwdArgs& a, const ScanTBwdOut& wo, const ScanTSeg& sg, int phase, aum_stream_t s) {
+    if (a.flags & AUM_SCAN_DELTA_ACTIVATED) {
+        if constexpr (sizeof(T) == 2) {
+            switch (phase) {
+                case 0: return launch_scant_seg_bwd<T, 0, SCANT_SP_ACT, true>(a, wo, sg, s);
+                case 1: return launch_scant_seg_bwd<T, 1, SCANT_SP_ACT, true>(a, wo, sg, s);
+                case 2: return launch_scant_seg_bwd<T, 2, SCANT_SP_ACT, true>(a, wo, sg, s);
+            }
+        }
+        return AUM_E_UNSUPPORTED;
+    }
     const int key = ((a.flags & AUM_SCAN_SOFTPLUS) ? 2 : 0) | (a.z ? 1 : 0);
     switch (phase * 4 + key) {
-#define AUM_TMS(P, K) case (P) * 4 + (K): return launch_scant_seg_bwd<T, P, ((K) & 2) != 0, ((K) & 1) != 0>(a, wo, sg, s);
+#define AUM_TMS(P, K) case (P) * 4 + (K): return launch_scant_seg_bwd<T, P, ((K) & 2) ? SCANT_SP_IN : SCANT_SP_NONE, ((K) & 1) != 0>(a, wo, sg, s);
 #define AUM_TMS4(P) AUM_TMS(P, 0) AUM_TMS(P, 1) AUM_TMS(P, 2) AUM_TMS(P, 3)
         AUM_TMS4(0) AUM_TMS4(1) AUM_TMS4(2)
 #undef AUM_TMS4
@@ -231,12 +246,22 @@
     return dtype == AUM_F32 ? scant_ck_rows<float>() : (dtype == AUM_BF16 || dtype == AUM_F16) ? scant_ck_rows<bf16_t>() : 0;
 }
 
+static bool scan_tm_act_ok(uint32_t flags, int32_t dtype, const void* z) { return !(flags & AUM_SCAN_DELTA_ACTIVATED) || (dtype != AUM_F32 && z); }
+static AumScanTmFwdArgs scan_tm_fwd_resolve(const AumScanTmFwdArgs& a) {
+    AumScanTmFwdArgs r = a;
+    if (a.flags & AUM_SCAN_DELTA_ACTIVATED) {
+        r.delta_bias = nullptr;
+        r.flags &= ~(AUM_SCAN_SOFTPLUS | AUM_SCAN_DELTA_ACTIVATED);
+    }
+    return r;
+}
 static int scan_tm_fwd_check(const AumScanTmFwdArgs* a) {
     if (!a) return AUM_E_NULL;
     if (!a->u || !a->delta || !a->B || !a->C || !a->A || !a->out) return AUM_E_NULL;
     if (a->batch <= 0 || a->dim <= 0 || a->len <= 0 || a->dstate <= 0) return AUM_E_SHAPE;
     if (a->dtype < 0 || a->dtype > 2) return AUM_E_DTYPE;
     if (!scant_supported(a->dim, a->dstate)) return AUM_E_UNSUPPORTED;
+    if (!scan_tm_act_ok(a->flags, a->dtype, a->z)) return AUM_E_UNSUPPORTED;
     if (a->A_b && (a->flags & AUM_SCAN_REVERSE)) return AUM_E_UNSUPPORTED;
     if (a->dtype != AUM_F32) {
         if ((a->B_bs | a->B_ts | a->C_bs | a->C_ts) & 1) return AUM_E_UNSUPPORTED;
@@ -259,10 +284,11 @@
     const int rc = scan_tm_fwd_check(a);
     if (rc != AUM_OK) return rc;
     aum_stream_t s = (aum_stream_t)stream;
-    switch (a->dtype) {
-        case AUM_F32: return scan_tm_fwd_f32(*a, s);
-        case AUM_BF16: return scan_tm_fwd_bf16(*a, s);
-        default: return scan_tm_fwd_f16(*a, s);
+    const AumScanTmFwdArgs k = scan_tm_fwd_resolve(*a);
+    switch (k.dtype) {
+        case AUM_F32: return scan_tm_fwd_f32(k, s);
+        case AUM_BF16: return scan_tm_fwd_bf16(k, s);
+        default: return scan_tm_fwd_f16(k, s);
     }
 }
 static int scan_tm_seg_fwd_any(const AumScanTmFwdArgs& a, const ScanTSeg& sg, int phase, aum_stream_t s) {
@@ -292,14 +318,15 @@
     sg.seg_len = scant_seg_len(a->len, sa->segments);
     sg.dir0 = 0;
     sg.ndl = bidir ? 2 : 1;
-    int r = scan_tm_seg_fwd_any(*a, sg, 3, s);
+    const AumScanTmFwdArgs k = scan_tm_fwd_resolve(*a);
+    int r = scan_tm_seg_fwd_any(k, sg, 3, s);
     if (r != AUM_OK) return r;
     sg.ndl = 1;
-    if (!bidir) return scan_tm_seg_fwd_any(*a, sg, 0, s);
-    r = scan_tm_seg_fwd_any(*a, sg, 1, s);
+    if (!bidir) return scan_tm_seg_fwd_any(k, sg, 0, s);
+    r = scan_tm_seg_fwd_any(k, sg, 1, s);
     if (r != AUM_OK) return r;
     sg.dir0 = 1;
-    return scan_tm_seg_fwd_any(*a, sg, 2, s);
+    return scan_tm_seg_fwd_any(k, sg, 2, s);
 }
 AUM_API int64_t aum_scan_tm_workspace_bytes(int32_t batch, int32_t dim, int32_t len, int32_t dstate, int32_t bidirectional) {
     if (batch <= 0 || dim <= 0 || len <= 0 || dstate <= 0 || !scant_supported(dim, dstate)) return 0;
@@ -406,6 +433,7 @@
     if (a->dtype < 0 || a->dtype > 2) return AUM_E_DTYPE;
     if (!scant_supported(a->dim, a->dstate)) return AUM_E_UNSUPPORTED;
     if (a->A_b && (a->flags & AUM_SCAN_REVERSE)) return AUM_E_UNSUPPORTED;
+    if (!scan_tm_act_ok(a->flags, a->dtype, a->z)) return AUM_E_UNSUPPORTED;
     const int64_t es = a->dtype == AUM_F32 ? 4 : 2, lim = ((int64_t)1 << 31) - 1;
     if (a->dtype != AUM_F32) {
         if ((a->B_bs | a->B_ts | a->C_bs | a->C_ts) & 1) return AUM_E_UNSUPPORTED;
@@ -440,12 +468,15 @@
     wo.trace = reinterpret_cast<unsigned long long*>(ws + L.trace);
 #endif
     aum_stream_t s = (aum_stream_t)stream;
+    const bool act = (a->flags & AUM_SCAN_DELTA_ACTIVATED) != 0;
+    AumScanTmBwdArgs k = *a;
+    if (act) k.delta_bias = nullptr;
     int rc = AUM_OK;
     if (nseg == 1) {
-        switch (a->dtype) {
-            case AUM_F32: rc = scan_tm_bwd_f32(*a, wo, s); break;
-            case AUM_BF16: rc = scan_tm_bwd_bf16(*a, wo, s); break;
-            default: rc = scan_tm_bwd_f16(*a, wo, s); break;
+        switch (k.dtype) {
+            case AUM_F32: rc = scan_tm_bwd_f32(k, wo, s); break;
+            case AUM_BF16: rc = scan_tm_bwd_bf16(k, wo, s); break;
+            default: rc = scan_tm_bwd_f16(k, wo, s); break;
         }
     } else {
         ScanTSeg sg;
@@ -464,24 +495,24 @@
             f.A = a->A; f.A_b = a->A_b; f.delta_bias = a->delta_bias;
             f.out = a->du; f.out_bs = a->du_bs; f.out_ts = a->du_ts;
             f.batch = a->batch; f.dim = a->dim; f.len = a->len; f.dstate = a->dstate; f.dtype = a->dtype; f.flags = a->flags;
-            rc = scan_tm_seg_fwd_any(f, sg, 4, s);
+            rc = scan_tm_seg_fwd_any(scan_tm_fwd_resolve(f), sg, 4, s);
             if (rc != AUM_OK) return rc;
         }
         sg.ndl = 1;
         for (int d = 0; d < (bidir ? 2 : 1) && rc == AUM_OK; ++d) {
             sg.dir0 = d;
             const int phase = bidir ? 1 + d : 0;
-            switch (a->dtype) {
-                case AUM_F32: rc = scan_tm_seg_bwd_f32(*a, wo, sg, phase, s); break;
-                case AUM_BF16: rc = scan_tm_seg_bwd_bf16(*a, wo, sg, phase, s); break;
-                default: rc = scan_tm_seg_bwd_f16(*a, wo, sg, phase, s); break;
+            switch (k.dtype) {
+                case AUM_F32: rc = scan_tm_seg_bwd_f32(k, wo, sg, phase, s); break;
+                case AUM_BF16: rc = scan_tm_seg_bwd_bf16(k, wo, sg, phase, s); break;
+                default: rc = scan_tm_seg_bwd_f16(k, wo, sg, phase, s); break;
             }
         }
     }
     if (rc != AUM_OK) return rc;
     ScanTReduceArgs r;
     r.ws = ws;
-    r.dBC = a->dBC; r.dA = a->dA; r.dA_b = a->dA_b; r.dD = a->D ? a->dD : nullptr; r.dbias = a->delta_bias ? a->ddelta_bias : nullptr;
+    r.dBC = a->dBC; r.dA = a->dA; r.dA_b = a->dA_b; r.dD = a->D ? a->dD : nullptr; r.dbias = a->delta_bias || act ? a->ddelta_bias : nullptr;
     r.o_dA = L.dA; r.o_dD = L.dD; r.o_dbias = L.dbias;
     r.A = a->A; r.A_b = a->A_b; r.dAx = a->dA_xA; r.dAx_b = a->A_b ? a->dA_b_xA : nullptr;
     r.batch = a->batch; r.pbatch = a->batch * nseg; r.dim = a->dim; r.len = a->len; r.dstate = a->dstate; r.nparts = L.nparts; r.ndir = L.ndir; r.nsum = scant_dbc_rows_to_sum(L.nparts, bidir);
diff --git a/audio-mamba-aum_amd/csrc/gemm.hip b/audio-mamba-aum_amd/csrc/gemm.hip
--- a/audio-mamba-aum_amd/csrc/gemm.hip
+++ b/audio-mamba-aum_amd/csrc/gemm.hip
@@ -87,17 +87,18 @@
 }
 
 
-template <int NW, int NC> static void xdt_launch_nc(const AumXdtArgs& g, hipStream_t s) {
+template <int NW, int NC, bool SP> static void xdt_launch_nc(const AumXdtArgs& g, hipStream_t s) {
     const dim3 grid((unsigned)((g.ntok + NW * XDT_TOK_W - 1) / (NW * XDT_TOK_W))), block(NW * 64);
     const bool bf = g.dtype == AUM_BF16, one = g.rank <= 32;
-    if (bf && one) hipLaunchKernelGGL((aumx::k_xdt_tm_fwd<true, 1, NW, NC>), grid, block, 0, s, g);
-    else if (bf) hipLaunchKernelGGL((aumx::k_xdt_tm_fwd<true, 2, NW, NC>), grid, block, 0, s, g);
-    else if (one) hipLaunchKernelGGL((aumx::k_xdt_tm_fwd<false, 1, NW, NC>), grid, block, 0, s, g);
-    else hipLaunchKernelGGL((aumx::k_xdt_tm_fwd<false, 2, NW, NC>), grid, block, 0, s, g);
+    if (bf && one) hipLaunchKernelGGL((aumx::k_xdt_tm_fwd<true, 1, NW, NC, SP>), grid, block, 0, s, g);
+    else if (bf) hipLaunchKernelGGL((aumx::k_xdt_tm_fwd<true, 2, NW, NC, SP>), grid, block, 0, s, g);
+    else if (one) hipLaunchKernelGGL((aumx::k_xdt_tm_fwd<false, 1, NW, NC, SP>), grid, block, 0, s, g);
+    else hipLaunchKernelGGL((aumx::k_xdt_tm_fwd<false, 2, NW, NC, SP>), grid, block, 0, s, g);
 }
 template <int NW> static void xdt_launch(const AumXdtArgs& g, hipStream_t s) {
-    if (g.ncols == XDT_COLS) xdt_launch_nc<NW, XDT_COLS>(g, s);
-    else xdt_launch_nc<NW, XDT_COLS_SMALL>(g, s);
+    const bool sp = (g.flags & AUM_XDT_DELTA_SOFTPLUS) != 0;
+    if (g.ncols == XDT_COLS) sp ? xdt_launch_nc<NW, XDT_COLS, true>(g, s) : xdt_launch_nc<NW, XDT_COLS, false>(g, s);
+    else sp ? xdt_launch_nc<NW, XDT_COLS_SMALL, true>(g, s) : xdt_launch_nc<NW, XDT_COLS_SMALL, false>(g, s);
 }
 
 extern "C" int aum_xdt_tm_fwd(const AumXdtArgs* p, void* stream) {
diff --git a/audio-mamba-aum_amd/csrc/scan_tm_kernels.h b/audio-mamba-aum_amd/csrc/scan_tm_kernels.h
--- a/audio-mamba-aum_amd/csrc/scan_tm_kernels.h
+++ b/audio-mamba-aum_amd/csrc/scan_tm_kernels.h
@@ -594,13 +594,14 @@
     unsigned long long* trace;
 };
 
+constexpr int SCANT_SP_NONE = 0, SCANT_SP_IN = 1, SCANT_SP_ACT = 2;
 #ifndef AUM_SCANT_TAIL2
 #define AUM_SCANT_TAIL2 1
 #endif
 #ifndef AUM_SCANT_BABL
 #define AUM_SCANT_BABL 0
 #endif
-template <class T, int N, int PHASE, bool SP, bool HAS_Z>
+template <class T, int N, int PHASE, int SP, bool HAS_Z>
 AUM_DEV void scant_bwd_run(const AumScanTmBwdArgs& p, const ScanTBwdOut& wo, int b, int e0, int dir, int part, int t0, int tstep, int it0,
                            int it1, const float* Aptr, float dmul, vf16& hh, vf16& dAacc, vf& dDacc, vf& dbacc, float* lds,
                            unsigned long long* tacc = nullptr) {
@@ -789,7 +790,7 @@
                 const int s0 = 2 * i, s1 = 2 * i + 1;
                 const vf2 us = mk2(raw_to_f32<T>(ru[s0]), raw_to_f32<T>(ru[s1]));
                 vf2 d = mk2(raw_to_f32<T>(rd[s0]), raw_to_f32<T>(rd[s1])) + bias2;
-                if (SP) d = vsoftplus2(d);
+                if (SP == SCANT_SP_IN) d = vsoftplus2(d);
                 Pd[i] = d;
                 Pu[i] = d * us;
                 const vf2 go = mk2(raw_to_f32<T>(rg[s0]), raw_to_f32<T>(rg[s1]));
@@ -968,7 +969,7 @@
                         du = du + mk2(raw_to_f32<T>(rpu[s0]), raw_to_f32<T>(rpu[s1]));
                         dd = dd + mk2(raw_to_f32<T>(rpd[s0]), raw_to_f32<T>(rpd[s1]));
                     }
-                    if (SP) dd = dd * (one2 - vexp2_2(dls * spl2(splat(-LOG2E))));
+                    if (SP != SCANT_SP_NONE) dd = dd * (one2 - vexp2_2(dls * spl2(splat(-LOG2E))));
                     dbacc = dbacc + lo2(dd);
                     dbacc = dbacc + hi2(dd);
                 }
@@ -994,7 +995,7 @@
                             du = du + raw_to_f32<T>(rpu[s]);
                             dd = dd + raw_to_f32<T>(rpd[s]);
                         }
-                        if (SP) dd = dd * (splat(1.f) - vexp2(dls * (-LOG2E)));
+                        if (SP != SCANT_SP_NONE) dd = dd * (splat(1.f) - vexp2(dls * (-LOG2E)));
                         dbacc = dbacc + dd;
                     }
                     lds_write_elem<T>(t_du, off, du);
@@ -1027,7 +1028,7 @@
 #undef AUM_TMB_STAMP
 }
 
-template <class T, bool SP, bool HAS_Z, bool BIDIR>
+template <class T, int SP, bool HAS_Z, bool BIDIR>
 AUM_DEV void scant_bwd(const AumScanTmBwdArgs& p, const ScanTBwdOut& wo, int wg, float* lds, unsigned long long* tacc = nullptr) {
     constexpr int N = SCANT_N;
     constexpr int NW = SCANT_NW;
@@ -1114,7 +1115,7 @@
     }
 }
 
-template <class T, int PHASE, bool SP, bool HAS_Z>
+template <class T, int PHASE, int SP, bool HAS_Z>
 AUM_DEV void scant_seg_bwd(const AumScanTmBwdArgs& p, const ScanTBwdOut& wo, const ScanTSeg& sg, int wg, float* lds) {
     constexpr int N = SCANT_N;
     constexpr int NW = SCANT_NW;
diff --git a/audio-mamba-aum_amd/csrc/xdt_args.h b/audio-mamba-aum_amd/csrc/xdt_args.h
--- a/audio-mamba-aum_amd/csrc/xdt_args.h
+++ b/audio-mamba-aum_amd/csrc/xdt_args.h
@@ -23,6 +23,8 @@
     if ((g.ncols != XDT_COLS && g.ncols != XDT_COLS_SMALL) || g.rank % 8 || g.rank > 64 || g.rank > g.ncols || g.dim % 256 || g.dim > XDT_MAX_DIM) return AUM_E_UNSUPPORTED;
     if (g.ldu % 8 || g.ldwx % 8 || g.ldwdt % 8 || g.ldx % 8 || g.ldd % 8) return AUM_E_UNSUPPORTED;
     if (((uintptr_t)g.u | (uintptr_t)g.wx | (uintptr_t)g.wdt | (uintptr_t)g.x_dbl | (uintptr_t)g.delta) & 15u) return AUM_E_UNSUPPORTED;
+    if ((g.flags & ~AUM_XDT_DELTA_SOFTPLUS) || (g.delta_bias && !(g.flags & AUM_XDT_DELTA_SOFTPLUS)) || ((uintptr_t)g.delta_bias & 15u))
+        return AUM_E_UNSUPPORTED;
     return AUM_OK;
 }
 inline int xdt_bwd_check(const AumXdtBwdArgs* p) {
diff --git a/audio-mamba-aum_amd/csrc/xdt_kernels.h b/audio-mamba-aum_amd/csrc/xdt_kernels.h
--- a/audio-mamba-aum_amd/csrc/xdt_kernels.h
+++ b/audio-mamba-aum_amd/csrc/xdt_kernels.h
@@ -2,6 +2,7 @@
 #include <hip/hip_runtime.h>
 #include <stdint.h>
 
+#include "wave.h"
 #include "xdt_args.h"
 
 namespace aumx {
@@ -70,7 +71,7 @@
     }
 }
 
-template <bool BF16, int KS, int NW, int NC>
+template <bool BF16, int KS, int NW, int NC, bool SOFTPLUS>
 __global__ __launch_bounds__(NW * 64, 1) void k_xdt_tm_fwd(AumXdtArgs g) {
     constexpr int NCF = (NC + 15) / 16;
     constexpr int XP = NC == 80 ? 176 : 144;
@@ -165,9 +166,14 @@
     char* ob = static_cast<char*>(g.delta) + ((t0 + rho) * g.ldd + kg * 8) * 2;
     const int64_t otf = (int64_t)16 * g.ldd * 2;
     const char* wdr = slab + ((rho >> 2) * 8 + (rho & 3)) * WDP + kg * 16;
+    static_assert((XDT_MAX_DIM / 2) / 4 <= XDT_WAVES_MIN * 64 && (XDT_MAX_DIM / 2) * (WDP + 4) <= slab_bytes(XDT_MAX_DIM), "bias staging");
+    const float* bl = reinterpret_cast<const float*>(slab + CH * WDP) + kg * 8;
     for (int half = 0; half < 2; ++half) {
         __syncthreads();
+        f4v bv = {0.f, 0.f, 0.f, 0.f};
+        if (SOFTPLUS && tid < CH / 4 && g.delta_bias) bv = *reinterpret_cast<const f4v*>(g.delta_bias + half * CH + tid * 4);
         stage_rows<NW * 64>(slab, WDP, static_cast<const char*>(g.wdt) + (int64_t)half * CH * g.ldwdt * 2, (int64_t)g.ldwdt * 2, CH, wchunks, tid);
+        if (SOFTPLUS && tid < CH / 4) *reinterpret_cast<f4v*>(slab + CH * WDP + tid * 16) = bv;
         __syncthreads();
         const int npairs = CH / 32;
 #pragma unroll 2
@@ -187,10 +193,22 @@
                     for (int ks = 0; ks < KS; ++ks) a2[j] = mfma<BF16>(wf[j][ks], xf[tf][ks], a2[j]);
                 if (tok_ok[tf]) {
                     u4v o;
-                    o.x = pack2<BF16>(a2[0][0], a2[0][1]);
-                    o.y = pack2<BF16>(a2[0][2], a2[0][3]);
-                    o.z = pack2<BF16>(a2[1][0], a2[1][1]);
-                    o.w = pack2<BF16>(a2[1][2], a2[1][3]);
+                    if constexpr (SOFTPLUS) {
+                        const f4v b0 = *reinterpret_cast<const f4v*>(bl + p * 32), b1 = *reinterpret_cast<const f4v*>(bl + p * 32 + 4);
+                        const aum::vf2 d0 = aum::vsoftplus2(aum::vf2{a2[0][0], a2[0][1]} + aum::vf2{b0[0], b0[1]});
+                        const aum::vf2 d1 = aum::vsoftplus2(aum::vf2{a2[0][2], a2[0][3]} + aum::vf2{b0[2], b0[3]});
+                        const aum::vf2 d2 = aum::vsoftplus2(aum::vf2{a2[1][0], a2[1][1]} + aum::vf2{b1[0], b1[1]});
+                        const aum::vf2 d3 = aum::vsoftplus2(aum::vf2{a2[1][2], a2[1][3]} + aum::vf2{b1[2], b1[3]});
+                        o.x = pack2<BF16>(d0[0], d0[1]);
+                        o.y = pack2<BF16>(d1[0], d1[1]);
+                        o.z = pack2<BF16>(d2[0], d2[1]);
+                        o.w = pack2<BF16>(d3[0], d3[1]);
+                    } else {
+                        o.x = pack2<BF16>(a2[0][0], a2[0][1]);
+                        o.y = pack2<BF16>(a2[0][2], a2[0][3]);
+                        o.z = pack2<BF16>(a2[1][0], a2[1][1]);
+                        o.w = pack2<BF16>(a2[1][2], a2[1][3]);
+                    }
                     *reinterpret_cast<u4v*>(ob + tf * otf + ((int64_t)half * CH + p * 32) * 2) = o;
                 }
             }
diff --git a/audio-mamba-aum_amd/mamba_ssm/ops/selective_scan_interface.py b/audio-mamba-aum_amd/mamba_ssm/ops/selective_scan_interface.py
--- a/audio-mamba-aum_amd/mamba_ssm/ops/selective_scan_interface.py
+++ b/audio-mamba-aum_amd/mamba_ssm/ops/selective_scan_interface.py
@@ -414,6 +414,7 @@
 _XDT_BWD_HIP = _dbg_env("AUM_XDT_BWD_LIB", "0") != "1"
 _XDT_HIP = _dbg_env("AUM_XDT_LIB", "0") != "1"
 _DTPROJ_HIP = _dbg_env("AUM_DTPROJ_LIB", "0") != "1"
+_DELTA_IN_XDT = _dbg_env("AUM_DELTA_IN_XDT", "1") != "0"
 _GEMM_MODE = _dbg_env("AUM_GEMM", "auto")
 if _GEMM_MODE not in ("auto", "hip", "lib"):
     raise ValueError("AUM_GEMM takes auto, hip or lib")
@@ -545,8 +546,11 @@
     conv_out = aum_hip.conv1d_tm_fwd(x, conv_w, conv1d_bias, True, reverse)
     conv2d = conv_out.view(Bsz * L, E)
     w_x, w_dt = x_proj_weight.to(conv2d.dtype), delta_proj_weight.to(conv2d.dtype)
+    act_delta = False
     if _XDT_HIP and conv2d.is_cuda and aum_hip.xdt_tm_supported(conv2d, w_x, w_dt):
-        x_dbl, delta = aum_hip.xdt_tm_fwd(conv2d, w_x, w_dt)
+        act_delta = _DELTA_IN_XDT and bool(delta_softplus)
+        x_dbl, delta = aum_hip.xdt_tm_fwd(conv2d, w_x, w_dt, delta_bias=delta_bias if act_delta else None,
+                                          delta_softplus=act_delta)
     else:
         x_dbl = torch.matmul(conv2d, w_x.t())
         delta = None
@@ -568,8 +572,9 @@
     cut = waves < (-(-_TM_MIN_WAVES * 4 // 3) if need_bwd and A_b is not None else _TM_MIN_WAVES)
     out_z, out_pre = aum_hip.scan_tm_fwd(conv_out, delta.view(Bsz, L, E), A, Bm, Cm, D, z, delta_bias, delta_softplus,
                                          reverse if A_b is None else False, A_b=A_b, want_out_pre=need_bwd, ckpt=ckpt,
-                                         segments=tm_segments(Bsz, E, L, A_b is not None, False, device=xz.device) if cut else 1)
-    ctx.tm_cut = cut
+                                         segments=tm_segments(Bsz, E, L, A_b is not None, False, device=xz.device) if cut else 1,
+                                         delta_activated=act_delta)
+    ctx.tm_cut, ctx.act_delta = cut, act_delta
     ctx.A_cached = (need_bwd and A.dtype == torch.float32 and A.is_contiguous() and A.data_ptr() in _A_CACHE_PTRS
                     and (A_b is None or (A_b.is_contiguous() and A_b.data_ptr() in _A_CACHE_PTRS)))
     ctx.tm = True
@@ -615,7 +620,7 @@
     g = aum_hip.scan_tm_bwd(conv_out, delta.view(Bsz, L, E), A, x3[:, :, R:R + N], x3[:, :, R + N:], D, z, delta_bias, dout_z, out_pre,
                             ckpt, ctx.delta_softplus, ctx.reverse if A_b is None else False, A_b=A_b, dz_out=dz,
                             segments=tm_segments(Bsz, E, L, A_b is not None, True, device=conv_out.device) if ctx.tm_cut else 1,
-                            want_dA_xA=ctx.A_cached,
+                            want_dA_xA=ctx.A_cached, delta_activated=ctx.act_delta,
                             param_out=dict(dD=H["D"], ddelta_bias=H["dt_bias"], dA_xA=H["A_log"], dA_b_xA=H["A_b_log"]))
     if ctx.A_cached:
         _da_xa_put(g["dA"], g["dA_xA"], A)
diff --git a/include/aum_hip.h b/include/aum_hip.h
--- a/include/aum_hip.h
+++ b/include/aum_hip.h
@@ -26,6 +26,7 @@
 #define AUM_SCAN_GENERIC 4u
 #define AUM_SCAN_ROWPAIR 8u
 #define AUM_SCAN_ACCUMULATE 16u
+#define AUM_SCAN_DELTA_ACTIVATED 32u
 #define AUM_CONV_SILU 1u
 #define AUM_CONV_REVERSE 2u
 #define AUM_CONV_GENERIC 4u
@@ -260,7 +261,10 @@
     int32_t dim, rank, ncols;
     int32_t ldu, ldwx, ldwdt, ldx, ldd;
     int32_t dtype;
+    const float* delta_bias;
+    uint32_t flags;
 } AumXdtArgs;
+#define AUM_XDT_DELTA_SOFTPLUS 1u
 int aum_xdt_tm_fwd(const AumXdtArgs* args, void* stream);
 
 typedef struct AumXdtBwdArgs {
```

Result: faster. 1091 clips/s, median of 6 (+2.0%).
